# hanruihua/NeuPAN

Hardware: AMD Instinct MI355X
Metric: MPC plans/sec (node), diff robot, 1k pts, T=10, K=10; ctrl L2 vs ref (higher is better)
Workload: dtype f32; 1 GPU; BASELINE.json configs[1]: batch=256 synthetic scenes/GPU, diff robot, 1000 pts, T=10, K=10 (iter_threshold=0), M=10, fp32 DUNE (MFMA) + fp64 QP; scenes_per_gpu=256, points=1000, T=10, K=10, M=10, batches_in_flight=40, chains=8, issue_threads=8

## Files before the change

neupan_amd/csrc/dune.hip:

```cpp
#include "pan_common.h"
#include <hip/hip_ext.h>
#include <algorithm>
#include <cstdlib>
#include <cstring>
#include "dune_device.h"

static int tiles_per_slice(const DevParams& P, int n_stride) {
  int n_use_max = n_stride < P.dune_max_num ? n_stride : P.dune_max_num;
  if (n_use_max < 1) n_use_max = 1;
  return (n_use_max + 31) / 32;
}

extern "C" hipError_t npa_launch_encode(const DevParams& P, const float* wpack, int batch, int scene0, int t0,
                                        int n_stride, const float* cur_s, const float* points, const float* vel,
                                        const int* n_points, const int* flags, unsigned* gkeys, const float* trig,
                                        int n_cu, int blocks_per_cu, int key_terms, hipStream_t stream,
                                        hipEvent_t ev_start, hipEvent_t ev_stop) {
  const int nsl = P.T + 1 - t0;
  const int tps = tiles_per_slice(P, n_stride);
  if (tps * 32 > P.key_stride) return hipErrorInvalidValue;
  const long long tiles = (long long)batch * nsl * tps;
  if (tiles >= (1ll << 31)) return hipErrorInvalidValue;
  const bool split = key_terms != 0, single = key_terms == 1;
  if (!split && blocks_per_cu > 4) blocks_per_cu = 4;
  static const bool small_only = getenv("NPA_ENC_WAVES") && atoi(getenv("NPA_ENC_WAVES")) == 4;
  int waves = (split && !small_only && P.E == 4 && tiles >= (long long)n_cu * 16 * 4) ? 16 : DUNE_WAVES;
  const int slots = waves >= 8 ? n_cu : n_cu * blocks_per_cu;
  int blocks = (int)((tiles + waves - 1) / waves);
  if (blocks > slots) blocks = slots;
  if (blocks < 1) blocks = 1;
  const size_t shmem = (11 * 32 + 8 * 32 + 8) * sizeof(float) + (split ? WP_KEY_LDS_FLOATS * sizeof(float) : 0);
  static const int chunk_env = getenv("NPA_ENC_CHUNK") ? atoi(getenv("NPA_ENC_CHUNK")) : 2;
  const int chunk = chunk_env < 1 ? 1 : chunk_env;
#define LAUNCH1(EE, SP, WV)                                                                                         \
  hipExtLaunchKernelGGL((dune_kernel<EE, SP, WV>), dim3(blocks), dim3(64 * WV), shmem, stream, ev_start, ev_stop, 0, \
                        P, wpack, n_stride, cur_s, points, vel, n_points, flags, gkeys, tps * 32, scene0, batch, t0, \
                        chunk, trig)
#define LAUNCH(EE)                                                                                                  \
  do {                                                                                                              \
    if (single) LAUNCH1(EE, 1, DUNE_WAVES);                                                                         \
    else if (split) LAUNCH1(EE, 3, DUNE_WAVES);                                                                     \
    else LAUNCH1(EE, 0, DUNE_WAVES);                                                                                \
  } while (0)
#define LAUNCH16(EE)                                                                                                \
  do {                                                                                                              \
    if (single && waves == 16) LAUNCH1(EE, 1, 16);                                                                  \
    else if (split && waves == 16) LAUNCH1(EE, 3, 16);                                                              \
    else LAUNCH(EE);                                                                                                \
  } while (0)
  switch (P.E) {
    case 3: LAUNCH(3); break;
    case 4: LAUNCH16(4); break;
    case 5: LAUNCH(5); break;
    case 6: LAUNCH(6); break;
    case 7: LAUNCH(7); break;
    case 8: LAUNCH(8); break;
    default: return hipErrorInvalidValue;
  }
#undef LAUNCH16
#undef LAUNCH
#undef LAUNCH1
  return hipGetLastError();
}

extern "C" hipError_t npa_launch_select(const DevParams& P, const float* wpack, int batch, int scene0, int t0,
                                        int n_stride, const float* cur_s, const float* points, const float* vel,
                                        const int* n_points, const int* flags, const unsigned* gkeys,
                                        const float* trig, float* mu_sorted, float* lam_sorted, float* pts_sorted,
                                        float* dist_sorted, int* count, int key_terms, float e0, unsigned* stats,
                                        int debug, hipStream_t stream, hipEvent_t ev_start, hipEvent_t ev_stop) {
  const int nsl = P.T + 1 - t0;
  const int tps = tiles_per_slice(P, n_stride);
  const int dbg = debug ? 2 : 1;
  const bool geo = key_terms == 4;
  const int approx = key_terms == 0 ? 0 : dbg;
  const size_t key_area = std::max<size_t>((size_t)tps * 32 * sizeof(unsigned), SEL_CAP * (NPA_MAX_E + 5 + 2) * sizeof(float));
  const size_t shmem = (11 * 32 + 8 * 32 + 8 + NPA_GEO_BANDS) * sizeof(float) + (SEL_CAP + NPA_MAX_M + 64) * sizeof(int) +
                       (key_area + 15) / 16 * 16;
#define LAUNCH1(EE, GG)                                                                                             \
  do {                                                                                                              \
    static NpaDeviceOnce big_lds;                                                                                   \
    int dev_ = 0;                                                                                                   \
    if (shmem > 60 * 1024 && big_lds.need(&dev_)) {                                                                 \
      hipError_t e_ = hipFuncSetAttribute(reinterpret_cast<const void*>(select_kernel<EE, GG>),                     \
                                          hipFuncAttributeMaxDynamicSharedMemorySize, 160 * 1024);                  \
      if (e_ != hipSuccess) return e_;                                                                              \
      big_lds.done(dev_);                                                                                           \
    }                                                                                                               \
    hipExtLaunchKernelGGL((select_kernel<EE, GG>), dim3(nsl, batch), dim3(64), shmem, stream, ev_start, ev_stop, 0, P,    \
                          wpack, n_stride, cur_s, points, vel, n_points, flags, gkeys, tps * 32, mu_sorted, lam_sorted, \
                          pts_sorted, dist_sorted, count, scene0, t0, approx, e0, stats, trig);                      \
  } while (0)
#ifdef NPA_EXPERIMENTS
#define LAUNCH(EE)                                                                                                  \
  do {                                                                                                              \
    if (geo) LAUNCH1(EE, true);                                                                                     \
    else LAUNCH1(EE, false);                                                                                        \
  } while (0)
#else
#define LAUNCH(EE)                                                                                                  \
  do {                                                                                                              \
    if (geo) return hipErrorInvalidValue;                                                                           \
    LAUNCH1(EE, false);                                                                                             \
  } while (0)
#endif
  switch (P.E) {
    case 3: LAUNCH(3); break;
    case 4: LAUNCH(4); break;
    case 5: LAUNCH(5); break;
    case 6: LAUNCH(6); break;
    case 7: LAUNCH(7); break;
    case 8: LAUNCH(8); break;
    default: return hipErrorInvalidValue;
  }
#undef LAUNCH
#undef LAUNCH1
  return hipGetLastError();
}

extern "C" hipError_t npa_launch_select_geo(const DevParams& P, const float* wpack, int batch, int scene0, int t0,
                                            int n_stride, const float* cur_s, const float* points, const float* vel,
                                            const int* n_points, const int* flags, const float* trig, float* mu_sorted,
                                            float* lam_sorted, float* pts_sorted, float* dist_sorted, int* count,
                                            unsigned* stats, int debug, unsigned* audit, unsigned audit_thresh,
                                            unsigned audit_seed, float margin_scale, int rows_bf16, hipStream_t stream,
                                            hipEvent_t ev_start, hipEvent_t ev_stop) {
  const int nsl = P.T + 1 - t0;
  int n_use_max = n_stride < P.dune_max_num ? n_stride : P.dune_max_num;
  if (n_use_max < 1) n_use_max = 1;
  const size_t n_pad = ((size_t)n_use_max + SEL2_TRIP - 1) / SEL2_TRIP * SEL2_TRIP;
  const size_t key_area = std::max<size_t>(n_pad * sizeof(unsigned), SEL_CAP * (NPA_MAX_E + 5 + 2) * sizeof(float));
  const size_t shmem = (11 * 32 + 8 * 32 + 8 + NPA_GEO_BANDS) * sizeof(float) + (2 * SEL_CAP + NPA_MAX_M) * sizeof(int) +
                       (key_area + 15) / 16 * 16;
  const int blocks = (batch + 7) / 8 * 8 * nsl;
#define LAUNCHG(EE, BB, KK)                                                                                         \
  do {                                                                                                              \
    static NpaDeviceOnce big_lds;                                                                                   \
    int dev_ = 0;                                                                                                   \
    if (shmem > 60 * 1024 && big_lds.need(&dev_)) {                                                                 \
      hipError_t e_ = hipFuncSetAttribute(reinterpret_cast<const void*>(select_geo_kernel<EE, BB, KK>),             \
                                          hipFuncAttributeMaxDynamicSharedMemorySize, 160 * 1024);                  \
      if (e_ != hipSuccess) return e_;                                                                              \
      big_lds.done(dev_);                                                                                           \
    }                                                                                                               \
    hipExtLaunchKernelGGL((select_geo_kernel<EE, BB, KK>), dim3(blocks), dim3(64), shmem, stream, ev_start, ev_stop, 0, P, wpack,  \
                          n_stride, cur_s, points, vel, n_points, flags, mu_sorted, lam_sorted, pts_sorted, dist_sorted, \
                          count, scene0, t0, nsl, batch, debug, stats, trig, audit, audit_thresh, audit_seed, margin_scale); \
  } while (0)
#define LAUNCH(EE)                                                                                                  \
  do {                                                                                                              \
    if (rows_bf16) return hipErrorInvalidValue;                                                                     \
    LAUNCHG(EE, false, false);                                                                                      \
  } while (0)
#define LAUNCHB(EE)                                                                                                 \
  do {                                                                                                              \
    if (rows_bf16 == 1) LAUNCHG(EE, true, false);                                                                   \
    else if (rows_bf16 == 2) LAUNCHG(EE, false, true);                                                              \
    else LAUNCHG(EE, false, false);                                                                                 \
  } while (0)
  switch (P.E) {
    case 3: LAUNCH(3); break;
    case 4: LAUNCHB(4); break;
    case 5: LAUNCH(5); break;
    case 6: LAUNCH(6); break;
    case 7: LAUNCH(7); break;
    case 8: LAUNCHB(8); break;
    default: return hipErrorInvalidValue;
  }
#undef LAUNCH
#undef LAUNCHB
#undef LAUNCHG
  return hipGetLastError();
}

extern "C" hipError_t npa_launch_select_geo_group(const DevParams& P, const SelGeoGroup& G, int n, int batch, int t0, int n_stride_max,
                                                  int debug, unsigned audit_thresh, float margin_scale, int rows_bf16,
                                                  hipStream_t stream, hipEvent_t ev_start, hipEvent_t ev_stop) {
  if (n < 1 || n > NPA_GROUP_MAX) return hipErrorInvalidValue;
  const int nsl = P.T + 1 - t0;
  int n_use_max = n_stride_max < P.dune_max_num ? n_stride_max : P.dune_max_num;
  if (n_use_max < 1) n_use_max = 1;
  const size_t n_pad = ((size_t)n_use_max + SEL2_TRIP - 1) / SEL2_TRIP * SEL2_TRIP;
  const size_t key_area = std::max<size_t>(n_pad * sizeof(unsigned), SEL_CAP * (NPA_MAX_E + 5 + 2) * sizeof(float));
  const size_t shmem = (11 * 32 + 8 * 32 + 8 + NPA_GEO_BANDS) * sizeof(float) + (2 * SEL_CAP + NPA_MAX_M) * sizeof(int) +
                       (key_area + 15) / 16 * 16;
  const int blocks = (batch + 7) / 8 * 8 * nsl;
#define LAUNCHG(EE, BB, KK)                                                                                         \
  do {                                                                                                              \
    static NpaDeviceOnce big_lds;                                                                                   \
    int dev_ = 0;                                                                                                   \
    if (shmem > 60 * 1024 && big_lds.need(&dev_)) {                                                                 \
      hipError_t e_ = hipFuncSetAttribute(reinterpret_cast<const void*>(select_geo_group_kernel<EE, BB, KK>),       \
                                          hipFuncAttributeMaxDynamicSharedMemorySize, 160 * 1024);                  \
      if (e_ != hipSuccess) return e_;                                                                              \
      big_lds.done(dev_);                                                                                           \
    }                                                                                                               \
    hipExtLaunchKernelGGL((select_geo_group_kernel<EE, BB, KK>), dim3(blocks, n), dim3(64), shmem, stream, ev_start, ev_stop, 0, P, G, \
                          t0, nsl, batch, debug, audit_thresh, margin_scale);                                       \
  } while (0)
  if (rows_bf16 == 1) return hipErrorInvalidValue;
  if (P.E == 4) { if (rows_bf16 == 2) LAUNCHG(4, false, true); else LAUNCHG(4, false, false); }
  else if (P.E == 8) { if (rows_bf16 == 2) LAUNCHG(8, false, true); else LAUNCHG(8, false, false); }
  else return hipErrorInvalidValue;
#undef LAUNCHG
  return hipGetLastError();
}
extern "C" int npa_select_geo_group_supported(int E) { return E == 4 || E == 8; }

template <int E>
__global__ __launch_bounds__(256) void geo_calib_kernel(DevParams P, const float* __restrict__ wpack, float half, int nside,
                                                        float inner, float shift, unsigned* __restrict__ out) {
  extern __shared__ __attribute__((aligned(16))) float smem[];
  float* vec = smem;
  float* w6 = vec + 11 * 32;
  float* b6 = w6 + 8 * 32;
  unsigned* tab = reinterpret_cast<unsigned*>(b6 + 8);
  const int tid = threadIdx.x, lane = tid & 63, j = lane & 31, hf = lane >> 5;
  for (int i = tid; i < 11 * 32 + 8 * 32 + 8; i += blockDim.x) smem[i] = wpack[WP_VEC + i];
  for (int i = tid; i < 2 * NPA_GEO_BANDS; i += blockDim.x) tab[i] = 0u;
  __syncthreads();
  WaveWeights W;
  load_weights(wpack, lane, W);
  const float step = 2.0f * half / (float)(nside - 1);
  const int tiles_x = nside >> 3, tiles_y = nside >> 2;
  const long long tiles = (long long)tiles_x * tiles_y;
  const long long wave = (long long)blockIdx.x * (blockDim.x >> 6) + (tid >> 6), nwave = (long long)gridDim.x * (blockDim.x >> 6);
  for (long long tile = wave; tile < tiles; tile += nwave) {
    const int ix = (int)(tile % tiles_x) * 8 + (j & 7), iy = (int)(tile / tiles_x) * 4 + (j >> 3);
    const float p0x = -half + step * ((float)ix + shift), p0y = -half + step * ((float)iy + shift);
    float me[E];
    encode_tile<E>(W, vec, w6, b6, p0x, p0y, lane, me);
    float de = 0.f;
#pragma unroll
    for (int e = 0; e < E; ++e) de = fmaf(me[e], __fsub_rn(fmaf(P.G[e][0], p0x, __fmul_rn(P.G[e][1], p0y)), P.h[e]), de);
    const float g = geo_dist<E>(P, p0x, p0y);
    float f = de - g;
    if (!(f == f)) f = 3.0e38f;
    const float fx = __shfl_down(f, 1, 64), fy = __shfl_down(f, 8, 64);
    if (hf == 0 && fmaxf(fabsf(p0x), fabsf(p0y)) >= inner) {
      const int band = npa_geo_band(g);
      atomicMax(&tab[band], __float_as_uint(fabsf(f)));
      float df = 0.f;
      if ((j & 7) < 7) df = fabsf(fx - f);
      if (j < 24) df = fmaxf(df, fabsf(fy - f));
      atomicMax(&tab[NPA_GEO_BANDS + band], __float_as_uint(df));
    }
  }
  __syncthreads();
  for (int i = tid; i < 2 * NPA_GEO_BANDS; i += blockDim.x)
    if (tab[i]) atomicMax(&out[i], tab[i]);
}

extern "C" hipError_t npa_launch_geo_calib(const DevParams& P, const float* wpack, int nside, float half, float inner,
                                           float shift, unsigned* out, int n_cu, hipStream_t stream) {
  const size_t shmem = (11 * 32 + 8 * 32 + 8 + 2 * NPA_GEO_BANDS) * sizeof(float);
  const int blocks = n_cu * 4;
#define LAUNCH(EE) hipLaunchKernelGGL((geo_calib_kernel<EE>), dim3(blocks), dim3(256), shmem, stream, P, wpack, half, nside, inner, shift, out)
  switch (P.E) {
    case 3: LAUNCH(3); break;
    case 4: LAUNCH(4); break;
    case 5: LAUNCH(5); break;
    case 6: LAUNCH(6); break;
    case 7: LAUNCH(7); break;
    case 8: LAUNCH(8); break;
    default: return hipErrorInvalidValue;
  }
#undef LAUNCH
  return hipGetLastError();
}

template <int E>
__global__ __launch_bounds__(256) void k16_calib_kernel(DevParams P, const float* __restrict__ wpack, float half, int nside, float inner,
                                                        unsigned* __restrict__ out) {
  extern __shared__ __attribute__((aligned(16))) float smem[];
  float* vec = smem;
  float* w6 = vec + 11 * 32;
  float* b6 = w6 + 8 * 32;
  unsigned* tab = reinterpret_cast<unsigned*>(b6 + 8);
  const int tid = threadIdx.x, lane = tid & 63, j = lane & 31, hf = lane >> 5;
  for (int i = tid; i < 11 * 32 + 8 * 32 + 8; i += blockDim.x) smem[i] = wpack[WP_VEC + i];
  for (int i = tid; i < NPA_GEO_BANDS; i += blockDim.x) tab[i] = 0u;
  __syncthreads();
  const float w1 = wpack[WP_W1 + lane];
  const float step = 2.0f * half / (float)(nside - 1);
  const int tiles_x = nside >> 3, tiles_y = nside >> 2;
  const long long tiles = (long long)tiles_x * tiles_y;
  const long long wave = (long long)blockIdx.x * (blockDim.x >> 6) + (tid >> 6), nwave = (long long)gridDim.x * (blockDim.x >> 6);
  for (long long tile = wave; tile < tiles; tile += nwave) {
    const int ix = (int)(tile % tiles_x) * 8 + (j & 7), iy = (int)(tile / tiles_x) * 4 + (j >> 3);
    const float p0x = -half + step * (float)ix, p0y = -half + step * (float)iy;
    float me[E], mb[E];
    encode_tile_stream<E>(w1, wpack + WP_WLS, vec, w6, b6, p0x, p0y, lane, me);
    encode_tile_bf16<E>(w1, wpack + WP_WB16, vec, w6, b6, p0x, p0y, lane, mb);
    float de = 0.f, db = 0.f;
#pragma unroll
    for (int e = 0; e < E; ++e) {
      const float tmp = __fsub_rn(fmaf(P.G[e][0], p0x, __fmul_rn(P.G[e][1], p0y)), P.h[e]);
      de = fmaf(me[e], tmp, de);
      db = fmaf(mb[e], tmp, db);
    }
    float f = fabsf(db - de);
    if (!(f == f)) f = 3.0e38f;
    if (hf == 0 && fmaxf(fabsf(p0x), fabsf(p0y)) >= inner) atomicMax(&tab[npa_geo_band(de)], __float_as_uint(f));
  }
  __syncthreads();
  for (int i = tid; i < NPA_GEO_BANDS; i += blockDim.x)
    if (tab[i]) atomicMax(&out[i], tab[i]);
}
extern "C" hipError_t npa_launch_k16_calib(const DevParams& P, const float* wpack, int nside, float half, float inner, unsigned* out,
                                           int n_cu, hipStream_t stream) {
  const size_t shmem = (11 * 32 + 8 * 32 + 8 + NPA_GEO_BANDS) * sizeof(float);
  const int blocks = n_cu * 4;
  if (P.E == 4) hipLaunchKernelGGL((k16_calib_kernel<4>), dim3(blocks), dim3(256), shmem, stream, P, wpack, half, nside, inner, out);
  else if (P.E == 8) hipLaunchKernelGGL((k16_calib_kernel<8>), dim3(blocks), dim3(256), shmem, stream, P, wpack, half, nside, inner, out);
  else return hipErrorInvalidValue;
  return hipGetLastError();
}

template <int E>
__global__ __launch_bounds__(256) void geo_table_nodes_kernel(DevParams P, const float* __restrict__ wpack, float* __restrict__ nodes) {
  extern __shared__ __attribute__((aligned(16))) float smem[];
  float* vec = smem;
  float* w6 = vec + 11 * 32;
  float* b6 = w6 + 8 * 32;
  const int tid = threadIdx.x, lane = tid & 63, j = lane & 31, hf = lane >> 5;
  for (int i = tid; i < 11 * 32 + 8 * 32 + 8; i += blockDim.x) smem[i] = wpack[WP_VEC + i];
  __syncthreads();
  const float w1 = wpack[WP_W1 + lane];
  constexpr int nside = NPA_TAB_N + 1, per = nside * nside, total = NPA_TAB_LEVELS * per;
  const int tiles = (total + 31) / 32;
  const int wave = blockIdx.x * (blockDim.x >> 6) + (tid >> 6), nwave = gridDim.x * (blockDim.x >> 6);
  for (int tile = wave; tile < tiles; tile += nwave) {
    const int n = tile * 32 + j, nc = n < total ? n : total - 1;
    const int lvl = nc / per, r = nc - lvl * per, iy = r / nside, ix = r - iy * nside;
    const float half = wpack[WP_TABH + 2] * (lvl == 0 ? 1.0f : (lvl == 1 ? 4.0f : (lvl == 2 ? 16.0f : 64.0f)));
    const float step = 2.0f * half / (float)NPA_TAB_N;
    const float p0x = wpack[WP_TABH] + fmaf(step, (float)ix, -half), p0y = wpack[WP_TABH + 1] + fmaf(step, (float)iy, -half);
    float me[E];
    encode_tile_stream<E>(w1, wpack + WP_WLS, vec, w6, b6, p0x, p0y, lane, me);
    float de = 0.f;
#pragma unroll
    for (int e = 0; e < E; ++e) de = fmaf(me[e], __fsub_rn(fmaf(P.G[e][0], p0x, __fmul_rn(P.G[e][1], p0y)), P.h[e]), de);
    if (hf == 0 && n < total) nodes[n] = de - geo_key<E>(P, p0x, p0y);
  }
}
__global__ void geo_table_pack_kernel(const float* __restrict__ nodes, float* __restrict__ wpack) {
  const int c = blockIdx.x * blockDim.x + threadIdx.x;
  constexpr int N = NPA_TAB_N, nside = N + 1;
  if (c >= NPA_TAB_LEVELS * N * N) return;
  const int lvl = c / (N * N), r = c - lvl * N * N, iy = r / N, ix = r - iy * N;
  const float* nl = nodes + (size_t)lvl * nside * nside;
  typedef _Float16 h2_t __attribute__((ext_vector_type(2)));
  union { unsigned u; h2_t h; } lo, hi;
  lo.h[0] = (_Float16)nl[iy * nside + ix]; lo.h[1] = (_Float16)nl[iy * nside + ix + 1];
  hi.h[0] = (_Float16)nl[(iy + 1) * nside + ix]; hi.h[1] = (_Float16)nl[(iy + 1) * nside + ix + 1];
  reinterpret_cast<uint2*>(wpack + WP_TAB)[c] = make_uint2(lo.u, hi.u);
}
extern "C" hipError_t npa_launch_geo_table(const DevParams& P, float* wpack, float* nodes, int n_cu, hipStream_t stream) {
  const size_t shmem = (11 * 32 + 8 * 32 + 8) * sizeof(float);
  const int blocks = n_cu * 4;
#define LAUNCH(EE) hipLaunchKernelGGL((geo_table_nodes_kernel<EE>), dim3(blocks), dim3(256), shmem, stream, P, wpack, nodes)
  switch (P.E) {
    case 4: LAUNCH(4); break;
    case 8: LAUNCH(8); break;
    default: return hipErrorInvalidValue;
  }
#undef LAUNCH
  hipError_t e = hipGetLastError();
  if (e != hipSuccess) return e;
  const int cells = NPA_TAB_LEVELS * NPA_TAB_N * NPA_TAB_N;
  hipLaunchKernelGGL(geo_table_pack_kernel, dim3((cells + 255) / 256), dim3(256), 0, stream, nodes, wpack);
  return hipGetLastError();
}
template <int E>
__global__ __launch_bounds__(256) void ktab_calib_kernel(DevParams P, const float* __restrict__ wpack, float half, int nside, float inner,
                                                         float cx, float cy, unsigned* __restrict__ out) {
  extern __shared__ __attribute__((aligned(16))) float smem[];
  float* vec = smem;
  float* w6 = vec + 11 * 32;
  float* b6 = w6 + 8 * 32;
  unsigned* tab = reinterpret_cast<unsigned*>(b6 + 8);
  const int tid = threadIdx.x, lane = tid & 63, j = lane & 31, hf = lane >> 5;
  for (int i = tid; i < 11 * 32 + 8 * 32 + 8; i += blockDim.x) smem[i] = wpack[WP_VEC + i];
  for (int i = tid; i < NPA_GEO_BANDS; i += blockDim.x) tab[i] = 0u;
  __syncthreads();
  const float w1 = wpack[WP_W1 + lane];
  const float step = 2.0f * half / (float)(nside - 1);
  const int tiles_x = nside >> 3, tiles_y = nside >> 2;
  const long long tiles = (long long)tiles_x * tiles_y;
  const long long wave = (long long)blockIdx.x * (blockDim.x >> 6) + (tid >> 6), nwave = (long long)gridDim.x * (blockDim.x >> 6);
  for (long long tile = wave; tile < tiles; tile += nwave) {
    const int ix = (int)(tile % tiles_x) * 8 + (j & 7), iy = (int)(tile / tiles_x) * 4 + (j >> 3);
    const float qx = -half + step * (float)ix, qy = -half + step * (float)iy;
    const float p0x = cx + qx, p0y = cy + qy;
    float me[E];
    encode_tile_stream<E>(w1, wpack + WP_WLS, vec, w6, b6, p0x, p0y, lane, me);
    float de = 0.f;
#pragma unroll
    for (int e = 0; e < E; ++e) de = fmaf(me[e], __fsub_rn(fmaf(P.G[e][0], p0x, __fmul_rn(P.G[e][1], p0y)), P.h[e]), de);
    const float kc = geo_key<E>(P, p0x, p0y) + geo_tab_corr(wpack, p0x, p0y);
    float f = fabsf(kc - de);
    if (!(f == f)) f = 3.0e38f;
    if (hf == 0 && fmaxf(fabsf(qx), fabsf(qy)) >= inner) atomicMax(&tab[npa_geo_band(kc)], __float_as_uint(f));
  }
  __syncthreads();
  for (int i = tid; i < NPA_GEO_BANDS; i += blockDim.x)
    if (tab[i]) atomicMax(&out[i], tab[i]);
}
extern "C" hipError_t npa_launch_ktab_calib(const DevParams& P, const float* wpack, int nside, float half, float inner, float cx, float cy,
                                            unsigned* out, int n_cu, hipStream_t stream) {
  const size_t shmem = (11 * 32 + 8 * 32 + 8 + NPA_GEO_BANDS) * sizeof(float);
  const int blocks = n_cu * 4;
#define LAUNCH(EE) hipLaunchKernelGGL((ktab_calib_kernel<EE>), dim3(blocks), dim3(256), shmem, stream, P, wpack, half, nside, inner, cx, cy, out)
  switch (P.E) {
    case 4: LAUNCH(4); break;
    case 8: LAUNCH(8); break;
    default: return hipErrorInvalidValue;
  }
#undef LAUNCH
  return hipGetLastError();
}

template <int E, int TERMS>
__global__ __launch_bounds__(256) void key_calib_kernel(DevParams P, const float* __restrict__ wpack, float lo, float step,
                                                        int nside, unsigned* __restrict__ out) {
  extern __shared__ __attribute__((aligned(16))) float smem[];
  float* vec = smem;
  float* w6 = vec + 11 * 32;
  float* b6 = w6 + 8 * 32;
  float* wb = b6 + 8;
  const int tid = threadIdx.x, lane = tid & 63, j = lane & 31, hf = lane >> 5;
  for (int i = tid; i < 11 * 32 + 8 * 32 + 8; i += blockDim.x) smem[i] = wpack[WP_VEC + i];
  for (int i = tid; i < WP_KEY_LDS_FLOATS; i += blockDim.x) wb[i] = wpack[WP_BF + i];
  __syncthreads();
  const f16x8* wbf = reinterpret_cast<const f16x8*>(wb);
  WaveWeights W;
  load_weights(wpack, lane, W);
  const float kw1 = wpack[WP_KW1 + lane];
  const int tile = blockIdx.x * (blockDim.x >> 6) + (tid >> 6);
  const int n = tile * 32 + j, total = nside * nside;
  const int nc = n < total ? n : total - 1;
  const float p0x = lo + step * (float)(nc % nside), p0y = lo + step * (float)(nc / nside);
  float mk[E], me[E];
  encode_tile_keys<E, TERMS>(kw1, wbf, vec, w6, b6, p0x, p0y, lane, mk);
  encode_tile<E>(W, vec, w6, b6, p0x, p0y, lane, me);
  float dk = 0.f, de = 0.f;
#pragma unroll
  for (int e = 0; e < E; ++e) {
    const float tmp = __fsub_rn(fmaf(P.G[e][0], p0x, __fmul_rn(P.G[e][1], p0y)), P.h[e]);
    dk = e < P.E ? fmaf(mk[e], tmp, dk) : dk;
    de = e < P.E ? fmaf(me[e], tmp, de) : de;
  }
  float rel = fabsf(dk - de) / (1.0f + fabsf(de));
  if (!(rel == rel)) rel = 1e30f;
  if (hf == 0 && n < total) atomicMax(out, __float_as_uint(rel));
}

extern "C" hipError_t npa_launch_key_calib(const DevParams& P, const float* wpack, int key_terms, int nside, float half,
                                           unsigned* out, hipStream_t stream) {
  const int tiles = (nside * nside + 31) / 32, blocks = (tiles + 3) / 4;
  const float lo = -half, step = 2.0f * half / (float)(nside - 1);
  const size_t shmem = (11 * 32 + 8 * 32 + 8 + WP_KEY_LDS_FLOATS) * sizeof(float);
#define LAUNCH(EE)                                                                                                   \
  do {                                                                                                               \
    if (key_terms == 1) hipLaunchKernelGGL((key_calib_kernel<EE, 1>), dim3(blocks), dim3(256), shmem, stream, P, wpack, lo, step, nside, out); \
    else hipLaunchKernelGGL((key_calib_kernel<EE, 3>), dim3(blocks), dim3(256), shmem, stream, P, wpack, lo, step, nside, out); \
  } while (0)
  if (P.E < 3 || P.E > NPA_MAX_E) return hipErrorInvalidValue;
  LAUNCH(NPA_MAX_E);
#undef LAUNCH
  return hipGetLastError();
}

__global__ void trig_kernel(const float* __restrict__ cur_s, int nscene, int T, float* __restrict__ trig) {
  const int i = blockIdx.x * blockDim.x + threadIdx.x;
  if (i >= nscene * (T + 1)) return;
  const int b = i / (T + 1), t = i - b * (T + 1);
  float c, s;
  npa_trig(cur_s[(size_t)b * 3 * (T + 1) + 2 * (T + 1) + t], c, s);
  trig[2 * (size_t)i] = c;
  trig[2 * (size_t)i + 1] = s;
}
extern "C" hipError_t npa_launch_trig(const float* cur_s, int batch, int T, float* trig, hipStream_t stream) {
  const int n = batch * (T + 1);
  hipLaunchKernelGGL(trig_kernel, dim3((n + 255) / 256), dim3(256), 0, stream, cur_s, batch, T, trig);
  return hipGetLastError();
}
```

neupan_amd/csrc/dune_device.h:

```cpp
#pragma once

typedef float f32x16 __attribute__((ext_vector_type(16)));

#define DUNE_THREADS 256
#define DUNE_WAVES 4

#define WSYNC()                                              \
  do {                                                       \
    __builtin_amdgcn_fence(__ATOMIC_SEQ_CST, "wavefront");   \
    __builtin_amdgcn_wave_barrier();                         \
  } while (0)

__device__ __forceinline__ float pair_sum(float x) {
  auto r = __builtin_amdgcn_permlane32_swap(__float_as_uint(x), __float_as_uint(x), false, false);
  return __uint_as_float(r[0]) + __uint_as_float(r[1]);
}

__device__ __forceinline__ float tanh_scaled(float y) {
  float e = __builtin_amdgcn_exp2f(y);
  return fmaf(-2.0f, __builtin_amdgcn_rcpf(e + 1.0f), 1.0f);
}

__device__ __forceinline__ void load_vec16(const float* v, int hf, float out[16]) {
#pragma unroll
  for (int q = 0; q < 4; ++q) {
    float4 t = *reinterpret_cast<const float4*>(v + 8 * q + 4 * hf);
    out[4 * q + 0] = t.x; out[4 * q + 1] = t.y; out[4 * q + 2] = t.z; out[4 * q + 3] = t.w;
  }
}

template <bool PERM>
__device__ __forceinline__ void load_vec16x(const float* v, int hf, float out[16]) {
  if constexpr (!PERM) {
    load_vec16(v, hf, out);
  } else {
#pragma unroll
    for (int h2 = 0; h2 < 2; ++h2)
#pragma unroll
      for (int qq = 0; qq < 2; ++qq) {
        const float4 t = *reinterpret_cast<const float4*>(v + 16 * h2 + 8 * hf + 4 * qq);
        out[2 * (4 * qq + 0) + h2] = t.x; out[2 * (4 * qq + 1) + h2] = t.y; out[2 * (4 * qq + 2) + h2] = t.z; out[2 * (4 * qq + 3) + h2] = t.w;
      }
  }
}
template <bool PERM = false>
__device__ __forceinline__ f32x16 bias_init(const float* v, int hf) {
  float b[16];
  load_vec16x<PERM>(v, hf, b);
  f32x16 acc;
#pragma unroll
  for (int r = 0; r < 16; ++r) acc[r] = b[r];
  return acc;
}

typedef float f32x4 __attribute__((ext_vector_type(4)));
__device__ __forceinline__ float quad_sum(float x) {
  auto r = __builtin_amdgcn_permlane16_swap(__float_as_uint(x), __float_as_uint(x), false, false);
  return pair_sum(__uint_as_float(r[0]) + __uint_as_float(r[1]));
}

template <bool PERM = false>
__device__ __forceinline__ void ln_tanh(f32x16 acc, const float* g, const float* be, int hf, float a[16]) {
  float se = acc[0], so = acc[1];
#pragma unroll
  for (int r = 2; r < 16; r += 2) { se += acc[r]; so += acc[r + 1]; }
  float mean = (pair_sum(se) + pair_sum(so)) * (1.0f / 32.0f);
  float qe = 0.f, qo = 0.f;
#pragma unroll
  for (int r = 0; r < 16; r += 2) {
    a[r] = acc[r] - mean; qe = fmaf(a[r], a[r], qe);
    a[r + 1] = acc[r + 1] - mean; qo = fmaf(a[r + 1], a[r + 1], qo);
  }
  float var = (pair_sum(qe) + pair_sum(qo)) * (1.0f / 32.0f);
  float ve = var + 1e-5f;
  float rstd = __builtin_amdgcn_rsqf(ve);
  rstd = rstd * fmaf(-0.5f * ve * rstd, rstd, 1.5f);
  if constexpr (PERM) {
#pragma unroll
    for (int h2 = 0; h2 < 2; ++h2)
#pragma unroll
      for (int qq = 0; qq < 2; ++qq) {
        const float4 gv = *reinterpret_cast<const float4*>(g + 16 * h2 + 8 * hf + 4 * qq);
        const float4 bv = *reinterpret_cast<const float4*>(be + 16 * h2 + 8 * hf + 4 * qq);
        const int r0 = 2 * (4 * qq) + h2;
        a[r0 + 0] = tanh_scaled(fmaf(a[r0 + 0] * rstd, gv.x, bv.x));
        a[r0 + 2] = tanh_scaled(fmaf(a[r0 + 2] * rstd, gv.y, bv.y));
        a[r0 + 4] = tanh_scaled(fmaf(a[r0 + 4] * rstd, gv.z, bv.z));
        a[r0 + 6] = tanh_scaled(fmaf(a[r0 + 6] * rstd, gv.w, bv.w));
      }
    return;
  }
#pragma unroll
  for (int qd = 0; qd < 4; ++qd) {
    float4 gv = *reinterpret_cast<const float4*>(g + 8 * qd + 4 * hf);
    float4 bv = *reinterpret_cast<const float4*>(be + 8 * qd + 4 * hf);
    a[4 * qd + 0] = tanh_scaled(fmaf(a[4 * qd + 0] * rstd, gv.x, bv.x));
    a[4 * qd + 1] = tanh_scaled(fmaf(a[4 * qd + 1] * rstd, gv.y, bv.y));
    a[4 * qd + 2] = tanh_scaled(fmaf(a[4 * qd + 2] * rstd, gv.z, bv.z));
    a[4 * qd + 3] = tanh_scaled(fmaf(a[4 * qd + 3] * rstd, gv.w, bv.w));
  }
}

__device__ __forceinline__ f32x16 layer32(const float (&w)[16], const float (&a)[16], f32x16 acc) {
#pragma unroll
  for (int r = 0; r < 16; ++r) acc = __builtin_amdgcn_mfma_f32_32x32x2f32(w[r], a[r], acc, 0, 0, 0);
  return acc;
}

typedef _Float16 f16x8 __attribute__((ext_vector_type(8)));
typedef _Float16 f16x2 __attribute__((ext_vector_type(2)));
typedef float f32x2_t __attribute__((ext_vector_type(2)));


template <bool RELU>
__device__ __forceinline__ void split2(const float (&a)[16], f16x8 (&x1)[2], f16x8 (&x2)[2]) {
#pragma unroll
  for (int p = 0; p < 8; ++p) {
    f32x2_t v = {a[2 * p], a[2 * p + 1]};
    if constexpr (RELU) {
      v.x = __int_as_float(max(__float_as_int(v.x), 0));
      v.y = __int_as_float(max(__float_as_int(v.y), 0));
    }
    const f16x2 b1 = __builtin_convertvector(v, f16x2);
    const f32x2_t r1 = v - __builtin_convertvector(b1, f32x2_t);
    const f16x2 b2 = __builtin_convertvector(r1, f16x2);
    const int s = p >> 2, q = (2 * p) & 7;
    x1[s][q] = b1.x; x1[s][q + 1] = b1.y;
    x2[s][q] = b2.x; x2[s][q + 1] = b2.y;
  }
}

template <bool RELU, int TERMS>
__device__ __forceinline__ f32x16 layer32_f16x2(const f16x8* wl, int lane, const float (&a)[16], f32x16 acc) {
  if constexpr (TERMS == 1) {
    f16x8 x[2];
#pragma unroll
    for (int p = 0; p < 8; ++p) {
      f16x2 b1 = __builtin_convertvector(f32x2_t{a[2 * p], a[2 * p + 1]}, f16x2);
      if constexpr (RELU) b1 = __builtin_elementwise_max(b1, f16x2{(_Float16)0.f, (_Float16)0.f});
      const int s = p >> 2, q = (2 * p) & 7;
      x[s][q] = b1.x; x[s][q + 1] = b1.y;
    }
#pragma unroll
    for (int s = 0; s < 2; ++s) acc = __builtin_amdgcn_mfma_f32_32x32x16_f16(wl[(0 * 2 + s) * 64 + lane], x[s], acc, 0, 0, 0);
    return acc;
  }
  f16x8 x1[2], x2[2];
  split2<RELU>(a, x1, x2);
#pragma unroll
  for (int s = 0; s < 2; ++s) {
    const f16x8 w1 = wl[(0 * 2 + s) * 64 + lane], w2 = wl[(1 * 2 + s) * 64 + lane];
    acc = __builtin_amdgcn_mfma_f32_32x32x16_f16(w2, x1[s], acc, 0, 0, 0);
    acc = __builtin_amdgcn_mfma_f32_32x32x16_f16(w1, x2[s], acc, 0, 0, 0);
    acc = __builtin_amdgcn_mfma_f32_32x32x16_f16(w1, x1[s], acc, 0, 0, 0);
  }
  return acc;
}

typedef float f32x2 __attribute__((ext_vector_type(2)));

__device__ __forceinline__ void ln_tanh_centred(f32x16 acc, const float* g, const float* be, int hf, float eps,
                                                float out_scale, float a[16]) {
  f32x2 q2 = {0.f, 0.f};
#pragma unroll
  for (int p = 0; p < 8; ++p) {
    const f32x2 v = {acc[2 * p], acc[2 * p + 1]};
    q2 = __builtin_elementwise_fma(v, v, q2);
  }
  const float ve = fmaf(pair_sum(q2.x + q2.y), 1.0f / 32.0f, eps);
  float rstd = __builtin_amdgcn_rsqf(ve);
  rstd = rstd * fmaf(-0.5f * ve * rstd, rstd, 1.5f);
  const f32x2 rs = {rstd, rstd}, one = {1.f, 1.f}, osc = {out_scale, out_scale}, mtwo = {-2.f * out_scale, -2.f * out_scale};
#pragma unroll
  for (int qd = 0; qd < 4; ++qd) {
    const float4 gv = *reinterpret_cast<const float4*>(g + 8 * qd + 4 * hf);
    const float4 bv = *reinterpret_cast<const float4*>(be + 8 * qd + 4 * hf);
#pragma unroll
    for (int hh = 0; hh < 2; ++hh) {
      const f32x2 x = {acc[4 * qd + 2 * hh], acc[4 * qd + 2 * hh + 1]};
      const f32x2 gg = hh ? f32x2{gv.z, gv.w} : f32x2{gv.x, gv.y};
      const f32x2 bb = hh ? f32x2{bv.z, bv.w} : f32x2{bv.x, bv.y};
      const f32x2 y = __builtin_elementwise_fma(x * rs, gg, bb);
      f32x2 e = {__builtin_amdgcn_exp2f(y.x), __builtin_amdgcn_exp2f(y.y)};
      e = e + one;
      const f32x2 r = {__builtin_amdgcn_rcpf(e.x), __builtin_amdgcn_rcpf(e.y)};
      const f32x2 th = __builtin_elementwise_fma(r, mtwo, osc);
      a[4 * qd + 2 * hh] = th.x; a[4 * qd + 2 * hh + 1] = th.y;
    }
  }
}

template <int E, int TERMS>
__device__ __forceinline__ void encode_tile_keys(float kw1, const f16x8* wbf, const float* vec, const float* w6,
                                                 const float* b6, float p0x, float p0y, int lane, float mu[E]) {
  const int hf = lane >> 5;
  const float* kvec = reinterpret_cast<const float*>(wbf) + WP_BF_FLOATS;
  const float* ksc = kvec + 5 * 32;
  constexpr int LSTR = 2 * 2 * 64;
  float a[16];
  {
    f32x16 acc = bias_init(kvec + 0 * 32, hf);
    acc = __builtin_amdgcn_mfma_f32_32x32x2f32(kw1, hf ? p0y : p0x, acc, 0, 0, 0);
    ln_tanh_centred(acc, vec + V_G1 * 32, vec + V_BE1 * 32, hf, ksc[0], ksc[3], a);
  }
  {
    f32x16 acc = layer32_f16x2<false, TERMS>(wbf + 0 * LSTR, lane, a, bias_init(kvec + 1 * 32, hf));
#pragma unroll
    for (int r = 0; r < 16; ++r) a[r] = acc[r];
  }
  {
    f32x16 acc = layer32_f16x2<true, TERMS>(wbf + 1 * LSTR, lane, a, bias_init(kvec + 2 * 32, hf));
    ln_tanh_centred(acc, vec + V_G2 * 32, vec + V_BE2 * 32, hf, ksc[1], ksc[4], a);
  }
  {
    f32x16 acc = layer32_f16x2<false, TERMS>(wbf + 2 * LSTR, lane, a, bias_init(kvec + 3 * 32, hf));
#pragma unroll
    for (int r = 0; r < 16; ++r) a[r] = acc[r];
  }
  {
    f32x16 acc = layer32_f16x2<true, TERMS>(wbf + 3 * LSTR, lane, a, bias_init(kvec + 4 * 32, hf));
    ln_tanh_centred(acc, vec + V_G3 * 32, vec + V_BE3 * 32, hf, ksc[2], ksc[5], a);
  }
#pragma unroll
  for (int e = 0; e < E; ++e) {
    float wv[16];
    load_vec16(w6 + e * 32, hf, wv);
    f32x2 s2 = {0.f, 0.f};
#pragma unroll
    for (int p = 0; p < 8; ++p)
      s2 = __builtin_elementwise_fma(f32x2{wv[2 * p], wv[2 * p + 1]}, f32x2{a[2 * p], a[2 * p + 1]}, s2);
    mu[e] = fmaxf(pair_sum(s2.x + s2.y) + b6[e], 0.f);
  }
}

struct WaveWeights {
  float w1;
  float wl[4][16];
};

template <int E>
__device__ __forceinline__ void encode_tile(const WaveWeights& W, const float* vec, const float* w6, const float* b6,
                                            float p0x, float p0y, int lane, float mu[E]) {
  const int hf = lane >> 5;
  auto layer = [&](int L, const float (&a_)[16], f32x16 acc) -> f32x16 { return layer32(W.wl[L], a_, acc); };
  float a[16];
  {
    f32x16 acc = bias_init(vec + V_B1 * 32, hf);
    acc = __builtin_amdgcn_mfma_f32_32x32x2f32(W.w1, hf ? p0y : p0x, acc, 0, 0, 0);
    ln_tanh(acc, vec + V_G1 * 32, vec + V_BE1 * 32, hf, a);
  }
  {
    f32x16 acc = layer(0, a, bias_init(vec + V_B2 * 32, hf));
#pragma unroll
    for (int r = 0; r < 16; ++r) a[r] = fmaxf(acc[r], 0.f);
  }
  {
    f32x16 acc = layer(1, a, bias_init(vec + V_B3 * 32, hf));
    ln_tanh(acc, vec + V_G2 * 32, vec + V_BE2 * 32, hf, a);
  }
  {
    f32x16 acc = layer(2, a, bias_init(vec + V_B4 * 32, hf));
#pragma unroll
    for (int r = 0; r < 16; ++r) a[r] = fmaxf(acc[r], 0.f);
  }
  {
    f32x16 acc = layer(3, a, bias_init(vec + V_B5 * 32, hf));
    ln_tanh(acc, vec + V_G3 * 32, vec + V_BE3 * 32, hf, a);
  }
#pragma unroll
  for (int e = 0; e < E; ++e) {
    float wv[16];
    load_vec16(w6 + e * 32, hf, wv);
    float se = 0.f, so = 0.f;
#pragma unroll
    for (int r = 0; r < 16; r += 2) { se = fmaf(wv[r], a[r], se); so = fmaf(wv[r + 1], a[r + 1], so); }
    mu[e] = fmaxf((pair_sum(se) + pair_sum(so)) + b6[e], 0.f);
  }
}

__device__ __forceinline__ void load_layer(const float* __restrict__ wls, int L, int lane, float (&w)[16]) {
  asm volatile("" : "+v"(lane));
  const float4* p = reinterpret_cast<const float4*>(wls + ((size_t)L * 64 + lane) * 16);
#pragma unroll
  for (int q = 0; q < 4; ++q) {
    const float4 v = p[q];
    w[4 * q] = v.x; w[4 * q + 1] = v.y; w[4 * q + 2] = v.z; w[4 * q + 3] = v.w;
  }
}
template <int E, bool PERM = false>
__device__ __forceinline__ void encode_tile_stream(float w1, const float* __restrict__ wls, const float* vec, const float* w6,
                                                   const float* b6, float p0x, float p0y, int lane, float mu[E]) {
  int hf = lane >> 5;
  if constexpr (PERM) asm volatile("" : "+v"(hf));
  float a[16], wa[16], wb[16];
  load_layer(wls, 0, lane, wa);
  __builtin_amdgcn_sched_barrier(0);
  {
    f32x16 acc = bias_init<PERM>(vec + V_B1 * 32, hf);
    acc = __builtin_amdgcn_mfma_f32_32x32x2f32(w1, hf ? p0y : p0x, acc, 0, 0, 0);
    ln_tanh<PERM>(acc, vec + V_G1 * 32, vec + V_BE1 * 32, hf, a);
  }
  __builtin_amdgcn_sched_barrier(0);
  load_layer(wls, 1, lane, wb);
  __builtin_amdgcn_sched_barrier(0);
  {
    f32x16 acc = layer32(wa, a, bias_init<PERM>(vec + V_B2 * 32, hf));
#pragma unroll
    for (int r = 0; r < 16; ++r) a[r] = fmaxf(acc[r], 0.f);
  }
  __builtin_amdgcn_sched_barrier(0);
  load_layer(wls, 2, lane, wa);
  __builtin_amdgcn_sched_barrier(0);
  {
    f32x16 acc = layer32(wb, a, bias_init<PERM>(vec + V_B3 * 32, hf));
    ln_tanh<PERM>(acc, vec + V_G2 * 32, vec + V_BE2 * 32, hf, a);
  }
  __builtin_amdgcn_sched_barrier(0);
  load_layer(wls, 3, lane, wb);
  __builtin_amdgcn_sched_barrier(0);
  {
    f32x16 acc = layer32(wa, a, bias_init<PERM>(vec + V_B4 * 32, hf));
#pragma unroll
    for (int r = 0; r < 16; ++r) a[r] = fmaxf(acc[r], 0.f);
  }
  __builtin_amdgcn_sched_barrier(0);
  {
    f32x16 acc = layer32(wb, a, bias_init<PERM>(vec + V_B5 * 32, hf));
    ln_tanh<PERM>(acc, vec + V_G3 * 32, vec + V_BE3 * 32, hf, a);
  }
  __builtin_amdgcn_sched_barrier(0);
#pragma unroll
  for (int e = 0; e < E; ++e) {
    float wv[16];
    load_vec16x<PERM>(w6 + e * 32, hf, wv);
    float se = 0.f, so = 0.f;
#pragma unroll
    for (int r = 0; r < 16; r += 2) { se = fmaf(wv[r], a[r], se); so = fmaf(wv[r + 1], a[r + 1], so); }
    mu[e] = fmaxf((pair_sum(se) + pair_sum(so)) + b6[e], 0.f);
  }
}

__device__ __forceinline__ f32x4 ld4(const float* p) {
  const float4 t = *reinterpret_cast<const float4*>(p);
  return f32x4{t.x, t.y, t.z, t.w};
}
__device__ __forceinline__ void ln_tanh16(f32x4 c0, f32x4 c1, const float* g, const float* be, int kq, float a[8]) {
  float s = c0[0];
  s += c0[1]; s += c0[2]; s += c0[3]; s += c1[0]; s += c1[1]; s += c1[2]; s += c1[3];
  const float mean = quad_sum(s) * (1.0f / 32.0f);
  float q = 0.f;
#pragma unroll
  for (int r = 0; r < 4; ++r) { a[r] = c0[r] - mean; q = fmaf(a[r], a[r], q); }
#pragma unroll
  for (int r = 0; r < 4; ++r) { a[4 + r] = c1[r] - mean; q = fmaf(a[4 + r], a[4 + r], q); }
  const float var = quad_sum(q) * (1.0f / 32.0f);
  const float ve = var + 1e-5f;
  float rstd = __builtin_amdgcn_rsqf(ve);
  rstd = rstd * fmaf(-0.5f * ve * rstd, rstd, 1.5f);
#pragma unroll
  for (int qd = 0; qd < 2; ++qd) {
    const float4 gv = *reinterpret_cast<const float4*>(g + 8 * kq + 4 * qd);
    const float4 bv = *reinterpret_cast<const float4*>(be + 8 * kq + 4 * qd);
    a[4 * qd + 0] = tanh_scaled(fmaf(a[4 * qd + 0] * rstd, gv.x, bv.x));
    a[4 * qd + 1] = tanh_scaled(fmaf(a[4 * qd + 1] * rstd, gv.y, bv.y));
    a[4 * qd + 2] = tanh_scaled(fmaf(a[4 * qd + 2] * rstd, gv.z, bv.z));
    a[4 * qd + 3] = tanh_scaled(fmaf(a[4 * qd + 3] * rstd, gv.w, bv.w));
  }
}
__device__ __forceinline__ void layer16(const float (&w)[16], const float (&a)[8], f32x4& c0, f32x4& c1) {
#pragma unroll
  for (int s = 0; s < 8; ++s) {
    c0 = __builtin_amdgcn_mfma_f32_16x16x4f32(w[2 * s], a[s], c0, 0, 0, 0);
    c1 = __builtin_amdgcn_mfma_f32_16x16x4f32(w[2 * s + 1], a[s], c1, 0, 0, 0);
  }
}
template <int E>
__device__ __forceinline__ void encode_tile16_stream(float w1a, float w1b, const float* __restrict__ wls16, const float* vec,
                                                     const float* w6, const float* b6, float p0x, float p0y, int lane, float mu[E]) {
  int kq = lane >> 4;
  asm volatile("" : "+v"(kq));
  const float* vq = vec + 8 * kq;
  float a[8], wa[16], wb[16];
  load_layer(wls16, 0, lane, wa);
  __builtin_amdgcn_sched_barrier(0);
  {
    f32x4 c0 = ld4(vq + V_B1 * 32), c1 = ld4(vq + V_B1 * 32 + 4);
    const float bx = kq == 0 ? p0x : (kq == 1 ? p0y : 0.f);
    c0 = __builtin_amdgcn_mfma_f32_16x16x4f32(w1a, bx, c0, 0, 0, 0);
    c1 = __builtin_amdgcn_mfma_f32_16x16x4f32(w1b, bx, c1, 0, 0, 0);
    ln_tanh16(c0, c1, vec + V_G1 * 32, vec + V_BE1 * 32, kq, a);
  }
  __builtin_amdgcn_sched_barrier(0);
  load_layer(wls16, 1, lane, wb);
  __builtin_amdgcn_sched_barrier(0);
  {
    f32x4 c0 = ld4(vq + V_B2 * 32), c1 = ld4(vq + V_B2 * 32 + 4);
    layer16(wa, a, c0, c1);
#pragma unroll
    for (int r = 0; r < 4; ++r) { a[r] = fmaxf(c0[r], 0.f); a[4 + r] = fmaxf(c1[r], 0.f); }
  }
  __builtin_amdgcn_sched_barrier(0);
  load_layer(wls16, 2, lane, wa);
  __builtin_amdgcn_sched_barrier(0);
  {
    f32x4 c0 = ld4(vq + V_B3 * 32), c1 = ld4(vq + V_B3 * 32 + 4);
    layer16(wb, a, c0, c1);
    ln_tanh16(c0, c1, vec + V_G2 * 32, vec + V_BE2 * 32, kq, a);
  }
  __builtin_amdgcn_sched_barrier(0);
  load_layer(wls16, 3, lane, wb);
  __builtin_amdgcn_sched_barrier(0);
  {
    f32x4 c0 = ld4(vq + V_B4 * 32), c1 = ld4(vq + V_B4 * 32 + 4);
    layer16(wa, a, c0, c1);
#pragma unroll
    for (int r = 0; r < 4; ++r) { a[r] = fmaxf(c0[r], 0.f); a[4 + r] = fmaxf(c1[r], 0.f); }
  }
  __builtin_amdgcn_sched_barrier(0);
  {
    f32x4 c0 = ld4(vq + V_B5 * 32), c1 = ld4(vq + V_B5 * 32 + 4);
    layer16(wb, a, c0, c1);
    ln_tanh16(c0, c1, vec + V_G3 * 32, vec + V_BE3 * 32, kq, a);
  }
  __builtin_amdgcn_sched_barrier(0);
#pragma unroll
  for (int e = 0; e < E; ++e) {
    const f32x4 w0 = ld4(w6 + e * 32 + 8 * kq), w1 = ld4(w6 + e * 32 + 8 * kq + 4);
    float s = 0.f;
#pragma unroll
    for (int r = 0; r < 4; ++r) s = fmaf(w0[r], a[r], s);
#pragma unroll
    for (int r = 0; r < 4; ++r) s = fmaf(w1[r], a[4 + r], s);
    mu[e] = fmaxf(quad_sum(s) + b6[e], 0.f);
  }
}

typedef __bf16 bf16x8 __attribute__((ext_vector_type(8)));
typedef __bf16 bf16x2 __attribute__((ext_vector_type(2)));
__device__ __forceinline__ f32x16 layer32_bf16(const bf16x8* __restrict__ wb, int L, int lane, const float (&a)[16], f32x16 acc) {
  bf16x8 x[2];
#pragma unroll
  for (int p = 0; p < 8; ++p) {
    const bf16x2 b = __builtin_convertvector(f32x2_t{a[2 * p], a[2 * p + 1]}, bf16x2);
    const int s = p >> 2, q = (2 * p) & 7;
    x[s][q] = b.x; x[s][q + 1] = b.y;
  }
#pragma unroll
  for (int s = 0; s < 2; ++s) acc = __builtin_amdgcn_mfma_f32_32x32x16_bf16(wb[(L * 2 + s) * 64 + lane], x[s], acc, 0, 0, 0);
  return acc;
}
template <int E>
__device__ __forceinline__ void encode_tile_bf16(float w1, const float* __restrict__ wb16, const float* vec, const float* w6,
                                                 const float* b6, float p0x, float p0y, int lane, float mu[E]) {
  const int hf = lane >> 5;
  const bf16x8* wb = reinterpret_cast<const bf16x8*>(wb16);
  float a[16];
  {
    f32x16 acc = bias_init(vec + V_B1 * 32, hf);
    acc = __builtin_amdgcn_mfma_f32_32x32x2f32(w1, hf ? p0y : p0x, acc, 0, 0, 0);
    ln_tanh(acc, vec + V_G1 * 32, vec + V_BE1 * 32, hf, a);
  }
  {
    f32x16 acc = layer32_bf16(wb, 0, lane, a, bias_init(vec + V_B2 * 32, hf));
#pragma unroll
    for (int r = 0; r < 16; ++r) a[r] = fmaxf(acc[r], 0.f);
  }
  {
    f32x16 acc = layer32_bf16(wb, 1, lane, a, bias_init(vec + V_B3 * 32, hf));
    ln_tanh(acc, vec + V_G2 * 32, vec + V_BE2 * 32, hf, a);
  }
  {
    f32x16 acc = layer32_bf16(wb, 2, lane, a, bias_init(vec + V_B4 * 32, hf));
#pragma unroll
    for (int r = 0; r < 16; ++r) a[r] = fmaxf(acc[r], 0.f);
  }
  {
    f32x16 acc = layer32_bf16(wb, 3, lane, a, bias_init(vec + V_B5 * 32, hf));
    ln_tanh(acc, vec + V_G3 * 32, vec + V_BE3 * 32, hf, a);
  }
#pragma unroll
  for (int e = 0; e < E; ++e) {
    float wv[16];
    load_vec16(w6 + e * 32, hf, wv);
    float se = 0.f, so = 0.f;
#pragma unroll
    for (int r = 0; r < 16; r += 2) { se = fmaf(wv[r], a[r], se); so = fmaf(wv[r + 1], a[r + 1], so); }
    mu[e] = fmaxf((pair_sum(se) + pair_sum(so)) + b6[e], 0.f);
  }
}

__device__ __forceinline__ unsigned ordered_key(float d) {
  if (d != d) return 0xFFFFFFFEu;
  unsigned b = __float_as_uint(d);
  return (b & 0x80000000u) ? ~b : (b | 0x80000000u);
}

template <int CTRL>
__device__ __forceinline__ unsigned long long dpp_u64(unsigned long long v) {
  unsigned lo = (unsigned)__builtin_amdgcn_update_dpp(0, (int)(unsigned)v, CTRL, 0xF, 0xF, false);
  unsigned hi = (unsigned)__builtin_amdgcn_update_dpp(0, (int)(unsigned)(v >> 32), CTRL, 0xF, 0xF, false);
  return ((unsigned long long)hi << 32) | lo;
}
__device__ __forceinline__ unsigned long long umin64(unsigned long long a, unsigned long long b) { return a < b ? a : b; }
__device__ __forceinline__ unsigned long long readlane_u64(unsigned long long v, int l) {
  unsigned lo = __builtin_amdgcn_readlane((unsigned)v, l), hi = __builtin_amdgcn_readlane((unsigned)(v >> 32), l);
  return ((unsigned long long)hi << 32) | lo;
}
__device__ __forceinline__ unsigned long long wave_min_u64(unsigned long long v) {
  v = umin64(v, dpp_u64<0xB1>(v));
  v = umin64(v, dpp_u64<0x4E>(v));
  v = umin64(v, dpp_u64<0x141>(v));
  v = umin64(v, dpp_u64<0x140>(v));
  return umin64(umin64(readlane_u64(v, 0), readlane_u64(v, 16)), umin64(readlane_u64(v, 32), readlane_u64(v, 48)));
}

struct SliceFrame {
  float c, s, tx, ty;
  float tstep;
  float rg[2][NPA_MAX_E];
};

__device__ __forceinline__ int src_index(int n, int n_raw, int n_use) {
  if (n_use >= n_raw) return n;
  if (n == n_use - 1) return n_raw - 1;
  double step = (double)(n_raw - 1) / (double)(n_use - 1);
  return (int)((double)n * step);
}

template <int E>
__device__ __forceinline__ void load_frame(const DevParams& P, const float* __restrict__ cur_s,
                                           const float* __restrict__ trig, int b, int t, SliceFrame& F) {
  const int T = P.T;
  const float* s = cur_s + (size_t)b * 3 * (T + 1);
  F.tx = s[t];
  F.ty = s[(T + 1) + t];
  F.c = trig[((size_t)b * (T + 1) + t) * 2];
  F.s = trig[((size_t)b * (T + 1) + t) * 2 + 1];
  F.tstep = (float)t;
#pragma unroll
  for (int e = 0; e < E; ++e) {
    F.rg[0][e] = fmaf(-F.c, P.G[e][0], __fmul_rn(F.s, P.G[e][1]));
    F.rg[1][e] = fmaf(-F.s, P.G[e][0], -__fmul_rn(F.c, P.G[e][1]));
  }
  auto uni = [](float v) { return __uint_as_float(__builtin_amdgcn_readfirstlane(__float_as_uint(v))); };
  F.c = uni(F.c); F.s = uni(F.s); F.tx = uni(F.tx); F.ty = uni(F.ty); F.tstep = uni(F.tstep);
#pragma unroll
  for (int e = 0; e < E; ++e) { F.rg[0][e] = uni(F.rg[0][e]); F.rg[1][e] = uni(F.rg[1][e]); }
}

template <int E, int SPLIT>
__device__ __forceinline__ void point_features(const DevParams& P, const SliceFrame& F, const WaveWeights& W,
                                               const f16x8* wbf, const float* vec, const float* w6, const float* b6,
                                               const float* px_row, const float* py_row, const float* vx_row,
                                               const float* vy_row, int src, int lane, float mu[E], float& gx,
                                               float& gy, float& lx, float& ly, float& dist) {
  gx = px_row[src];
  gy = py_row[src];
  if (vx_row) {
    gx = __fadd_rn(gx, __fmul_rn(F.tstep, __fmul_rn(vx_row[src], P.dt32)));
    gy = __fadd_rn(gy, __fmul_rn(F.tstep, __fmul_rn(vy_row[src], P.dt32)));
  }
  float dx = __fsub_rn(gx, F.tx), dy = __fsub_rn(gy, F.ty);
  float p0x = fmaf(F.c, dx, __fmul_rn(F.s, dy));
  float p0y = fmaf(F.c, dy, -__fmul_rn(F.s, dx));
  if constexpr (SPLIT != 0) encode_tile_keys<E, SPLIT>(W.w1, wbf, vec, w6, b6, p0x, p0y, lane, mu);
  else encode_tile<E>(W, vec, w6, b6, p0x, p0y, lane, mu);
  lx = 0.f; ly = 0.f; dist = 0.f;
#pragma unroll
  for (int e = 0; e < E; ++e) {
    lx = fmaf(F.rg[0][e], mu[e], lx);
    ly = fmaf(F.rg[1][e], mu[e], ly);
    float tmp = __fsub_rn(fmaf(P.G[e][0], p0x, __fmul_rn(P.G[e][1], p0y)), P.h[e]);
    dist = fmaf(mu[e], tmp, dist);
  }
}

template <int E, bool BF16 = false, bool PERM = false>
__device__ __forceinline__ void point_features_stream(const DevParams& P, const SliceFrame& F, float w1, const float* __restrict__ wls,
                                                      const float* vec, const float* w6, const float* b6, const float* px_row,
                                                      const float* py_row, const float* vx_row, const float* vy_row, int src,
                                                      int lane, float mu[E], float& gx, float& gy, float& lx, float& ly,
                                                      float& dist, float& p0x, float& p0y) {
  gx = px_row[src];
  gy = py_row[src];
  if (vx_row) {
    gx = __fadd_rn(gx, __fmul_rn(F.tstep, __fmul_rn(vx_row[src], P.dt32)));
    gy = __fadd_rn(gy, __fmul_rn(F.tstep, __fmul_rn(vy_row[src], P.dt32)));
  }
  float dx = __fsub_rn(gx, F.tx), dy = __fsub_rn(gy, F.ty);
  p0x = fmaf(F.c, dx, __fmul_rn(F.s, dy));
  p0y = fmaf(F.c, dy, -__fmul_rn(F.s, dx));
  if constexpr (BF16) encode_tile_bf16<E>(w1, wls, vec, w6, b6, p0x, p0y, lane, mu);
  else encode_tile_stream<E, PERM>(w1, wls, vec, w6, b6, p0x, p0y, lane, mu);
  lx = 0.f; ly = 0.f; dist = 0.f;
#pragma unroll
  for (int e = 0; e < E; ++e) {
    lx = fmaf(F.rg[0][e], mu[e], lx);
    ly = fmaf(F.rg[1][e], mu[e], ly);
    float tmp = __fsub_rn(fmaf(P.G[e][0], p0x, __fmul_rn(P.G[e][1], p0y)), P.h[e]);
    dist = fmaf(mu[e], tmp, dist);
  }
}

template <int E>
__device__ __forceinline__ void point_features_stream16(const DevParams& P, const SliceFrame& F, float w1a, float w1b,
                                                        const float* __restrict__ wls16, const float* vec, const float* w6,
                                                        const float* b6, const float* px_row, const float* py_row,
                                                        const float* vx_row, const float* vy_row, int src, int lane, float mu[E],
                                                        float& gx, float& gy, float& lx, float& ly, float& dist, float& p0x,
                                                        float& p0y) {
  gx = px_row[src];
  gy = py_row[src];
  if (vx_row) {
    gx = __fadd_rn(gx, __fmul_rn(F.tstep, __fmul_rn(vx_row[src], P.dt32)));
    gy = __fadd_rn(gy, __fmul_rn(F.tstep, __fmul_rn(vy_row[src], P.dt32)));
  }
  float dx = __fsub_rn(gx, F.tx), dy = __fsub_rn(gy, F.ty);
  p0x = fmaf(F.c, dx, __fmul_rn(F.s, dy));
  p0y = fmaf(F.c, dy, -__fmul_rn(F.s, dx));
  encode_tile16_stream<E>(w1a, w1b, wls16, vec, w6, b6, p0x, p0y, lane, mu);
  lx = 0.f; ly = 0.f; dist = 0.f;
#pragma unroll
  for (int e = 0; e < E; ++e) {
    lx = fmaf(F.rg[0][e], mu[e], lx);
    ly = fmaf(F.rg[1][e], mu[e], ly);
    float tmp = __fsub_rn(fmaf(P.G[e][0], p0x, __fmul_rn(P.G[e][1], p0y)), P.h[e]);
    dist = fmaf(mu[e], tmp, dist);
  }
}

__device__ __forceinline__ void load_weights(const float* __restrict__ wpack, int lane, WaveWeights& W) {
  W.w1 = wpack[WP_W1 + lane];
#pragma unroll
  for (int l = 0; l < 4; ++l)
#pragma unroll
    for (int r = 0; r < 16; ++r) W.wl[l][r] = wpack[WP_WL + (l * 16 + r) * 64 + lane];
}

template <int E, int SPLIT, int WAVES>
__global__ __attribute__((amdgpu_flat_work_group_size(64 * WAVES, 64 * WAVES), amdgpu_waves_per_eu(WAVES >= 8 ? 7 : ((SPLIT == 0 && E >= 6) ? 3 : 4))))
void dune_kernel(
    DevParams P, const float* __restrict__ wpack, int n_stride, const float* __restrict__ cur_s,
    const float* __restrict__ points, const float* __restrict__ vel, const int* __restrict__ n_points,
    const int* __restrict__ flags, unsigned* __restrict__ gkeys, int key_stride, int scene0, int nscene, int t0,
    int chunk, const float* __restrict__ trig) {
  extern __shared__ __attribute__((aligned(16))) float smem[];
  __shared__ int wg_ticket_s;
  int* wg_ticket = &wg_ticket_s;
  if (threadIdx.x == 0) wg_ticket_s = 0;
  float* vec = smem;
  float* w6 = vec + 11 * 32;
  float* b6 = w6 + 8 * 32;
  const int tid = threadIdx.x, lane = tid & 63;
  const int wave = __builtin_amdgcn_readfirstlane(tid >> 6);
  const int j = lane & 31, hf = lane >> 5;
  const int T = P.T;

  for (int i = tid; i < 11 * 32 + 8 * 32 + 8; i += 64 * WAVES) smem[i] = wpack[WP_VEC + i];
  WaveWeights W;
  const f16x8* wbf = nullptr;
  if constexpr (SPLIT != 0) {
    float* wb = b6 + 8;
    for (int i = tid; i < WP_KEY_LDS_FLOATS; i += 64 * WAVES) wb[i] = wpack[WP_BF + i];
    wbf = reinterpret_cast<const f16x8*>(wb);
    W.w1 = wpack[WP_KW1 + lane];
  } else {
    load_weights(wpack, lane, W);
  }
  __syncthreads();

  const int nsl = T + 1 - t0;
  const int tps = key_stride >> 5;
  const int total = nscene * nsl * tps;
  const int wg_lo = (int)((long long)total * blockIdx.x / gridDim.x);
  const int wg_hi = (int)((long long)total * (blockIdx.x + 1) / gridDim.x);
  int g = 0, hi = 0, sl = 0, tile = 0;
  int cur_sl = -1, n_raw = 0, n_use = 0, t = 0;
  bool skip = false;
  SliceFrame F;
  const float *px_row = nullptr, *py_row = nullptr, *vx_row = nullptr, *vy_row = nullptr;
  unsigned* key_row = nullptr;
#pragma unroll 1
  for (;; ++g, ++tile) {
    if (g >= hi) {
      int c = 0;
      if (lane == 0) c = atomicAdd(wg_ticket, chunk);
      g = wg_lo + __builtin_amdgcn_readfirstlane(c);
      if (g >= wg_hi) break;
      hi = g + chunk < wg_hi ? g + chunk : wg_hi;
      sl = (int)((unsigned)g / (unsigned)tps);
      tile = g - sl * tps;
    } else if (tile == tps) {
      tile = 0;
      ++sl;
    }
    if (sl != cur_sl) {
      cur_sl = sl;
      const int bl = (int)((unsigned)sl / (unsigned)nsl), b = bl + scene0;
      t = sl - bl * nsl + t0;
      n_raw = n_points ? n_points[b] : n_stride;
      n_raw = n_raw < 0 ? 0 : (n_raw > n_stride ? n_stride : n_raw);
      n_use = n_raw < P.dune_max_num ? n_raw : P.dune_max_num;
      skip = (flags && flags[b * 4 + 0]) || n_use <= 0;
      if (!skip) {
        load_frame<E>(P, cur_s, trig, b, t, F);
        px_row = points + (size_t)b * 2 * n_stride;
        py_row = px_row + n_stride;
        vx_row = vel ? vel + (size_t)b * 2 * n_stride : nullptr;
        vy_row = vel ? vx_row + n_stride : nullptr;
        key_row = gkeys + ((size_t)b * (T + 1) + t) * key_stride;
      }
    }
    if (skip || tile * 32 >= n_use) continue;
    {
      const int n = tile * 32 + j;
      const int nc = n < n_use ? n : n_use - 1;
      float mu[E], gx, gy, lx, ly, dist;
      point_features<E, SPLIT>(P, F, W, wbf, vec, w6, b6, px_row, py_row, vx_row, vy_row, src_index(nc, n_raw, n_use),
                               lane, mu, gx, gy, lx, ly, dist);
      if (hf == 0 && n < n_use) key_row[n] = ordered_key(dist);
    }
  }
}

template <int E>
__device__ __forceinline__ float geo_dist(const DevParams& P, float x, float y) {
  if (P.geo_rect) {
    const float dx = fmaxf(fabsf(x - P.rcx) - P.rhx, 0.f), dy = fmaxf(fabsf(y - P.rcy) - P.rhy, 0.f);
    return __builtin_sqrtf(fmaf(dx, dx, dy * dy));
  }
  float best = 3.0e38f;
  bool inside = true;
#pragma unroll
  for (int e = 0; e < E; ++e) {
    const float rx = x - P.pvx[e], ry = y - P.pvy[e];
    inside = inside && (fmaf(P.pdy[e], rx, -(P.pdx[e] * ry)) <= 0.f);
    float t = fmaf(rx, P.pdx[e], ry * P.pdy[e]) * P.pil[e];
    t = fminf(fmaxf(t, 0.f), 1.f);
    const float qx = fmaf(-t, P.pdx[e], rx), qy = fmaf(-t, P.pdy[e], ry);
    best = fminf(best, fmaf(qx, qx, qy * qy));
  }
  return inside ? 0.f : __builtin_sqrtf(best);
}

#define SEL_CAP 64
template <int E, bool GEO>
__global__ __attribute__((amdgpu_flat_work_group_size(64, 64), amdgpu_waves_per_eu(E <= 6 ? 4 : 3, E <= 6 ? 4 : 3))) void select_kernel(
    DevParams P, const float* __restrict__ wpack, int n_stride, const float* __restrict__ cur_s,
    const float* __restrict__ points, const float* __restrict__ vel, const int* __restrict__ n_points,
    const int* __restrict__ flags, const unsigned* __restrict__ gkeys, int key_stride,
    float* __restrict__ mu_sorted, float* __restrict__ lam_sorted, float* __restrict__ pts_sorted,
    float* __restrict__ dist_sorted, int* __restrict__ count, int scene0, int t0, int approx_keys, float e0,
    unsigned* __restrict__ stats, const float* __restrict__ trig) {
  extern __shared__ __attribute__((aligned(16))) float smem[];
  float* vec = smem;
  float* w6 = vec + 11 * 32;
  float* b6 = w6 + 8 * 32;
  float* etab = b6 + 8;
  int* sel = reinterpret_cast<int*>(etab + NPA_GEO_BANDS);
  unsigned* skey = reinterpret_cast<unsigned*>(sel + SEL_CAP);
  int* lst = reinterpret_cast<int*>(skey + NPA_MAX_M);
  constexpr int ROW_W = E + 5;
  unsigned* dkey = reinterpret_cast<unsigned*>(lst + 64);
  float* rows = reinterpret_cast<float*>(dkey);
  unsigned* rkey = reinterpret_cast<unsigned*>(rows + SEL_CAP * (NPA_MAX_E + 5));
  const int t = blockIdx.x + t0, b = blockIdx.y + scene0, lane = threadIdx.x;
  const int j = lane & 31, hf = lane >> 5;
  const int T = P.T, M = P.M;
  if (flags && flags[b * 4 + 0]) return;
  int n_raw = n_points ? n_points[b] : n_stride;
  n_raw = n_raw < 0 ? 0 : (n_raw > n_stride ? n_stride : n_raw);
  const int n_use = n_raw < P.dune_max_num ? n_raw : P.dune_max_num;
  const size_t orow = (size_t)b * (T + 1) + t;
  if (n_use <= 0) {
    if (lane == 0) count[orow] = 0;
    return;
  }
  for (int i = lane; i < 11 * 32 + 8 * 32 + 8; i += 64) smem[i] = wpack[WP_VEC16 + i];
  if constexpr (GEO)
    for (int i = lane; i < NPA_GEO_BANDS; i += 64) etab[i] = wpack[WP_GEO + i];
  SliceFrame F;
  load_frame<E>(P, cur_s, trig, b, t, F);
  const float* px_row = points + (size_t)b * 2 * n_stride;
  const float* py_row = px_row + n_stride;
  const float* vx_row = vel ? vel + (size_t)b * 2 * n_stride : nullptr;
  const float* vy_row = vel ? vx_row + n_stride : nullptr;
  if constexpr (GEO) {
    constexpr int KU = 4;
    auto key_of = [&](float gx, float gy, float vx, float vy) -> unsigned {
      if (vx_row) {
        gx = __fadd_rn(gx, __fmul_rn(F.tstep, __fmul_rn(vx, P.dt32)));
        gy = __fadd_rn(gy, __fmul_rn(F.tstep, __fmul_rn(vy, P.dt32)));
      }
      const float dx = __fsub_rn(gx, F.tx), dy = __fsub_rn(gy, F.ty);
      const float p0x = fmaf(F.c, dx, __fmul_rn(F.s, dy)), p0y = fmaf(F.c, dy, -__fmul_rn(F.s, dx));
      const bool calibrated = fmaxf(fabsf(p0x), fabsf(p0y)) <= P.geo_rcal;
      return calibrated ? __float_as_uint(geo_dist<E>(P, p0x, p0y)) : NPA_GEO_KEY_FAR;
    };
    for (int n0 = lane; n0 < n_use; n0 += 64 * KU) {
      float gx[KU], gy[KU], vx[KU], vy[KU];
#pragma unroll
      for (int u = 0; u < KU; ++u) {
        const int n = n0 + 64 * u;
        const int src = src_index(n < n_use ? n : n_use - 1, n_raw, n_use);
        gx[u] = px_row[src]; gy[u] = py_row[src];
        vx[u] = vx_row ? vx_row[src] : 0.f; vy[u] = vy_row ? vy_row[src] : 0.f;
      }
#pragma unroll
      for (int u = 0; u < KU; ++u) {
        const int n = n0 + 64 * u;
        if (n < n_use) dkey[n] = key_of(gx[u], gy[u], vx[u], vy[u]);
      }
    }
  } else {
    const unsigned* gk = gkeys + orow * key_stride;
    for (int n = lane; n < n_use; n += 64) dkey[n] = gk[n];
  }
  const float w1a = wpack[WP_W116 + lane], w1b = wpack[WP_W116 + 64 + lane];
  const float* wls16 = wpack + WP_WL16;
  WSYNC();

  const int msel = n_use < M ? n_use : M;
  unsigned last_key = 0;
  auto extract = [&]() {
    for (int m = 0; m < msel; ++m) {
      unsigned long long best = ~0ull;
      for (int n = lane; n < n_use; n += 64) best = umin64(best, ((unsigned long long)dkey[n] << 32) | (unsigned)n);
      best = wave_min_u64(best);
      const int idx = (int)(best & 0xFFFFFFFFu);
      last_key = (unsigned)(best >> 32);
      if (lane == 0) { sel[m] = idx; skey[m] = last_key; dkey[idx] = 0xFFFFFFFFu; }
      WSYNC();
    }
  };
  auto extract_short = [&]() -> bool {
    unsigned lmin = 0xFFFFFFFFu;
    for (int n = lane; n < n_use; n += 64) lmin = min(lmin, dkey[n]);
    unsigned bound = 0;
    for (int bit = 31; bit >= 0; --bit) {
      const unsigned trial = bound | ((1u << bit) - 1u);
      if (__popcll(__ballot(lmin <= trial)) < msel) bound |= 1u << bit;
    }
    int L = 0;
    for (int n0 = 0; n0 < n_use; n0 += 64) {
      const int n = n0 + lane;
      const bool hit = n < n_use && dkey[n] <= bound;
      const unsigned long long bal = __ballot(hit);
      const int pos = L + __builtin_amdgcn_mbcnt_hi((unsigned)(bal >> 32), __builtin_amdgcn_mbcnt_lo((unsigned)bal, 0));
      if (hit && pos < 64) lst[pos] = n;
      L += __popcll(bal);
    }
    if (L > 64 || L < msel) return false;
    WSYNC();
    const int idx = lane < L ? lst[lane] : 0;
    const unsigned long long v = lane < L ? (((unsigned long long)dkey[idx] << 32) | (unsigned)idx) : ~0ull;
    int rk = 0;
    for (int i = 0; i < L; ++i) rk += readlane_u64(v, i) < v ? 1 : 0;
    if (lane < L && rk < msel) { sel[rk] = idx; skey[rk] = (unsigned)(v >> 32); dkey[idx] = 0xFFFFFFFFu; }
    const unsigned long long lastb = __ballot(lane < L && rk == msel - 1);
    last_key = (unsigned)(readlane_u64(v, (int)__builtin_ctzll(lastb)) >> 32);
    WSYNC();
    return true;
  };
  if (!extract_short()) extract();
  int ncand = msel, fellback = 0;
  bool widen = false;
  unsigned thr = 0;
  float U = 0.f;
  if constexpr (GEO) {
    widen = n_use > msel;
    float hi = -1.f;
    if (lane < msel) {
      const unsigned k = skey[lane];
      const float g = __uint_as_float(k);
      hi = (k == NPA_GEO_KEY_FAR) ? __builtin_inff() : g + etab[npa_geo_band(g)];
    }
    for (int i = 0; i < msel; ++i) U = fmaxf(U, __uint_as_float(__builtin_amdgcn_readlane(__float_as_uint(hi), i)));
  } else {
    widen = approx_keys && msel == M && n_use > M && last_key < 0xFFFFFFFEu;
    if (widen) {
      const float dM = __uint_as_float((last_key & 0x80000000u) ? (last_key & 0x7FFFFFFFu) : ~last_key);
      thr = ordered_key(dM + 2.0f * e0 * (1.0f + fabsf(dM)));
    }
  }
  bool overflow = false, all = false;
  int total = 0, extra = 0;
  if (widen) {
    for (int n0 = 0; n0 < n_use; n0 += 64) {
      const int n = n0 + lane;
      bool hit = false;
      if (n < n_use) {
        const unsigned k = dkey[n];
        if constexpr (GEO) {
          const float g = __uint_as_float(k);
          hit = k != 0xFFFFFFFFu && (k == NPA_GEO_KEY_FAR || g - etab[npa_geo_band(g)] <= U);
        } else {
          hit = k <= thr;
        }
      }
      const unsigned long long bal = __ballot(hit);
      const int pos = extra + __builtin_amdgcn_mbcnt_hi((unsigned)(bal >> 32), __builtin_amdgcn_mbcnt_lo((unsigned)bal, 0));
      if (hit) dkey[pos] = (unsigned)n;
      extra += __popcll(bal);
    }
    WSYNC();
    if (msel + extra <= SEL_CAP) {
      if (lane < extra) sel[msel + lane] = (int)dkey[lane];
      ncand = msel + extra;
      WSYNC();
    } else {
      overflow = true;
      fellback = 1;
      all = 2 * extra + msel > n_use;
      total = all ? n_use : msel + extra;
    }
  }
  unsigned* ckey = dkey + extra;
  auto cand_index = [&](int q) { return all ? q : (q < msel ? sel[q] : (int)dkey[q - msel]); };
#pragma unroll 1
  for (int phase = overflow ? 0 : 1;; phase = 1) {
    const int cnt = phase == 0 ? total : ncand;
#pragma unroll 1
    for (int q0 = 0; q0 < cnt; q0 += 16) {
      const int q = q0 + (lane & 15), qc = q < cnt ? q : cnt - 1;
      const int idx = phase == 0 ? cand_index(qc) : sel[qc];
      float mu[E], gx, gy, lx, ly, dist, p0x, p0y;
      point_features_stream16<E>(P, F, w1a, w1b, wls16, vec, w6, b6, px_row, py_row, vx_row, vy_row,
                                 src_index(idx, n_raw, n_use), lane, mu, gx, gy, lx, ly, dist, p0x, p0y);
      if (lane < 16 && q < cnt) {
        const unsigned k = ordered_key(dist);
        if (phase == 0) {
          if (all) dkey[idx] = k;
          else ckey[q] = k;
        } else {
          float* r = rows + q * ROW_W;
#pragma unroll
          for (int e = 0; e < E; ++e) r[e] = mu[e];
          r[E] = lx; r[E + 1] = ly; r[E + 2] = gx; r[E + 3] = gy; r[E + 4] = dist;
          rkey[2 * q] = (unsigned)idx; rkey[2 * q + 1] = k;
        }
      }
    }
    WSYNC();
    if (phase == 1) break;
    if (stats && lane == 0) atomicAdd(stats, (unsigned)((total + 31) / 32));
    if (all) {
      extract();
    } else {
      int mywin = 0;
      for (int m2 = 0; m2 < msel; ++m2) {
        unsigned long long best = ~0ull;
        int bq = -1;
        for (int q = lane; q < total; q += 64) {
          const unsigned long long v = ((unsigned long long)ckey[q] << 32) | (unsigned)cand_index(q);
          if (v < best) { best = v; bq = q; }
        }
        const unsigned long long win = wave_min_u64(best);
        if (best == win && bq >= 0) ckey[bq] = 0xFFFFFFFFu;
        if (lane == m2) mywin = (int)(win & 0xFFFFFFFFu);
        WSYNC();
      }
      if (lane < msel) sel[lane] = mywin;
      WSYNC();
    }
    ncand = msel;
  }
  const bool mine = lane < ncand;
  const unsigned long long kx = mine ? (((unsigned long long)rkey[2 * lane + 1] << 32) | rkey[2 * lane]) : ~0ull;
  int rank = 0;
  for (int i = 0; i < ncand; ++i) rank += readlane_u64(kx, i) < kx ? 1 : 0;
  if (mine && rank < msel) {
    const float* r = rows + lane * ROW_W;
    auto put = [&](int q) {
      const size_t o = orow * M + q;
#pragma unroll
      for (int e = 0; e < E; ++e) mu_sorted[o * E + e] = r[e];
      lam_sorted[o * 2 + 0] = r[E]; lam_sorted[o * 2 + 1] = r[E + 1];
      pts_sorted[o * 2 + 0] = r[E + 2]; pts_sorted[o * 2 + 1] = r[E + 3];
      dist_sorted[o] = r[E + 4];
    };
    put(rank);
    if (rank == 0)
      for (int q = msel; q < M; ++q) put(q);
  }
  if (lane == 0) count[orow] = approx_keys == 2 ? (msel | (ncand << 8) | (fellback << 16)) : msel;
}

__device__ __forceinline__ float dpp_f32_b1(float v) { return __int_as_float(__builtin_amdgcn_update_dpp(0, __float_as_int(v), 0xB1, 0xF, 0xF, false)); }
__device__ __forceinline__ float wave_max_f32(float v) {
  v = fmaxf(v, dpp_f32_b1(v));
  v = fmaxf(v, __int_as_float(__builtin_amdgcn_update_dpp(0, __float_as_int(v), 0x4E, 0xF, 0xF, false)));
  v = fmaxf(v, __int_as_float(__builtin_amdgcn_update_dpp(0, __float_as_int(v), 0x141, 0xF, 0xF, false)));
  v = fmaxf(v, __int_as_float(__builtin_amdgcn_update_dpp(0, __float_as_int(v), 0x140, 0xF, 0xF, false)));
  auto rl = [&](int l) { return __uint_as_float(__builtin_amdgcn_readlane(__float_as_uint(v), l)); };
  return fmaxf(fmaxf(rl(0), rl(16)), fmaxf(rl(32), rl(48)));
}
template <int E, bool RECT>
__device__ __forceinline__ float geo_key_t(const DevParams& P, float x, float y) {
  if constexpr (RECT) {
    const float dx = fmaxf(fabsf(x - P.rcx) - P.rhx, 0.f), dy = fmaxf(fabsf(y - P.rcy) - P.rhy, 0.f);
    return __builtin_amdgcn_sqrtf(fmaf(dx, dx, dy * dy));
  } else {
    float best = 3.0e38f;
    bool inside = true;
#pragma unroll
    for (int e = 0; e < E; ++e) {
      const float rx = x - P.pvx[e], ry = y - P.pvy[e];
      inside = inside && (fmaf(P.pdy[e], rx, -(P.pdx[e] * ry)) <= 0.f);
      float t = fmaf(rx, P.pdx[e], ry * P.pdy[e]) * P.pil[e];
      t = fminf(fmaxf(t, 0.f), 1.f);
      const float qx = fmaf(-t, P.pdx[e], rx), qy = fmaf(-t, P.pdy[e], ry);
      best = fminf(best, fmaf(qx, qx, qy * qy));
    }
    return inside ? 0.f : __builtin_amdgcn_sqrtf(best);
  }
}
template <int E>
__device__ __forceinline__ float geo_key(const DevParams& P, float x, float y) {
  return P.geo_rect ? geo_key_t<E, true>(P, x, y) : geo_key_t<E, false>(P, x, y);
}

__device__ __forceinline__ float geo_tab_corr(const float* __restrict__ wpack, float x, float y) {
  const float cx = wpack[WP_TABH], cy = wpack[WP_TABH + 1], h0 = wpack[WP_TABH + 2], inv0 = wpack[WP_TABH + 3];
  const float rx = x - cx, ry = y - cy;
  const float a = fmaxf(fabsf(rx), fabsf(ry));
  const int lvl = a < h0 ? 0 : (a < 4.0f * h0 ? 1 : (a < 16.0f * h0 ? 2 : 3));
  const float sc = lvl == 0 ? 1.0f : (lvl == 1 ? 4.0f : (lvl == 2 ? 16.0f : 64.0f));
  const float half = h0 * sc, inv = inv0 * (1.0f / sc);
  const float fx = fminf(fmaxf((rx + half) * inv, 0.f), (float)NPA_TAB_N - 0.001f);
  const float fy = fminf(fmaxf((ry + half) * inv, 0.f), (float)NPA_TAB_N - 0.001f);
  const int ix = (int)fx, iy = (int)fy;
  const float tx = fx - (float)ix, ty = fy - (float)iy;
  const uint2 c = reinterpret_cast<const uint2*>(wpack + WP_TAB)[((size_t)lvl * NPA_TAB_N + iy) * NPA_TAB_N + ix];
  typedef _Float16 h2_t __attribute__((ext_vector_type(2)));
  union { unsigned u; h2_t h; } lo, hi;
  lo.u = c.x; hi.u = c.y;
  const float f00 = (float)lo.h[0], f10 = (float)lo.h[1], f01 = (float)hi.h[0], f11 = (float)hi.h[1];
  const float r0 = fmaf(tx, f10 - f00, f00), r1 = fmaf(tx, f11 - f01, f01);
  return fmaf(ty, r1 - r0, r0);
}

#define SEL2_TRIP 256
template <int E, bool RECT, bool VEL, bool DEC>
__device__ __forceinline__ unsigned key_pass(const DevParams& P, const SliceFrame& F, const float* px_row, const float* py_row,
                                             const float* vx_row, const float* vy_row, unsigned* dkey, int n_raw, int n_use,
                                             int n_pad, int lane) {
  const __amdgpu_buffer_rsrc_t rx = __builtin_amdgcn_make_buffer_rsrc(const_cast<float*>(px_row), 0, n_raw * 4, 0x00020000);
  const __amdgpu_buffer_rsrc_t ry = __builtin_amdgcn_make_buffer_rsrc(const_cast<float*>(py_row), 0, n_raw * 4, 0x00020000);
  const __amdgpu_buffer_rsrc_t rvx = __builtin_amdgcn_make_buffer_rsrc(const_cast<float*>(VEL ? vx_row : px_row), 0, n_raw * 4, 0x00020000);
  const __amdgpu_buffer_rsrc_t rvy = __builtin_amdgcn_make_buffer_rsrc(const_cast<float*>(VEL ? vy_row : py_row), 0, n_raw * 4, 0x00020000);
  const float tdt = F.tstep;
  unsigned lmin = 0xFFFFFFFFu;
  for (int n0 = 0; n0 < n_pad; n0 += SEL2_TRIP) {
    float gx[4], gy[4], vx[4], vy[4];
#pragma unroll
    for (int u = 0; u < 4; ++u) {
      const int n = n0 + lane + 64 * u;
      unsigned off = (unsigned)n * 4u;
      if constexpr (DEC) off = (unsigned)src_index(n < n_use ? n : n_use - 1, n_raw, n_use) * 4u;
      gx[u] = __uint_as_float(__builtin_amdgcn_raw_buffer_load_b32(rx, off, 0, 0));
      gy[u] = __uint_as_float(__builtin_amdgcn_raw_buffer_load_b32(ry, off, 0, 0));
      if constexpr (VEL) {
        vx[u] = __uint_as_float(__builtin_amdgcn_raw_buffer_load_b32(rvx, off, 0, 0));
        vy[u] = __uint_as_float(__builtin_amdgcn_raw_buffer_load_b32(rvy, off, 0, 0));
      }
    }
#pragma unroll
    for (int u = 0; u < 4; ++u) {
      const int n = n0 + lane + 64 * u;
      float x = gx[u], y = gy[u];
      if constexpr (VEL) {
        x = __fadd_rn(x, __fmul_rn(tdt, __fmul_rn(vx[u], P.dt32)));
        y = __fadd_rn(y, __fmul_rn(tdt, __fmul_rn(vy[u], P.dt32)));
      }
      const float dx = x - F.tx, dy = y - F.ty;
      const float p0x = fmaf(F.c, dx, F.s * dy), p0y = fmaf(F.c, dy, -(F.s * dx));
      unsigned k = __float_as_uint(geo_key_t<E, RECT>(P, p0x, p0y));
      k = n < n_use ? k : 0xFFFFFFFFu;
      dkey[n] = k;
      lmin = min(lmin, k);
    }
  }
  return lmin;
}

#define SEL2_TRIP 256
#ifdef NPA_SEL_PROF
#define SELP_WAVES 4096
__device__ unsigned long long npa_sel_prof[SELP_WAVES][16];
extern "C" int npa_dbg_sel_prof(unsigned long long* out16, int reset) {
  static unsigned long long host[SELP_WAVES][16];
  if (out16) {
    if (hipMemcpyFromSymbol(host, HIP_SYMBOL(npa_sel_prof), sizeof(host)) != hipSuccess) return -1;
    for (int i = 0; i < 16; ++i) { out16[i] = 0; for (int w = 0; w < SELP_WAVES; ++w) out16[i] += host[w][i]; }
  }
  if (reset) {
    memset(host, 0, sizeof(host));
    if (hipMemcpyToSymbol(HIP_SYMBOL(npa_sel_prof), host, sizeof(host)) != hipSuccess) return -1;
  }
  return 0;
}
#define SELP_DECL unsigned long long spt_ = __builtin_amdgcn_s_memtime(), sacc_[11] = {0, 0, 0, 0, 0, 0, 0, 0, 0, 0, 0}; const unsigned long long sp0_ = spt_
#define SELP(i) do { const unsigned long long n_ = __builtin_amdgcn_s_memtime(); sacc_[i] += n_ - spt_; spt_ = n_; } while (0)
#else
#define SELP_DECL
#define SELP(i)
#endif
template <int E, bool BF16 = false, bool KEYS16 = false>
__global__ __attribute__((amdgpu_flat_work_group_size(64, 64), amdgpu_waves_per_eu(E <= 6 ? 4 : 3, E <= 6 ? 4 : 3))) void select_geo_kernel(
    DevParams P, const float* __restrict__ wpack, int n_stride, const float* __restrict__ cur_s,
    const float* __restrict__ points, const float* __restrict__ vel, const int* __restrict__ n_points,
    const int* __restrict__ flags, float* __restrict__ mu_sorted, float* __restrict__ lam_sorted,
    float* __restrict__ pts_sorted, float* __restrict__ dist_sorted, int* __restrict__ count, int scene0, int t0, int nsl,
    int nscene, int debug, unsigned* __restrict__ stats, const float* __restrict__ trig, unsigned* __restrict__ audit,
    unsigned audit_thresh, unsigned audit_seed, float margin_scale) {
#include "select_geo_carve.inc"
  const int lane = threadIdx.x, j = lane & 31, hf = lane >> 5;
  SELP_DECL;
  const int w = blockIdx.x, xcd = w & 7, r_ = w >> 3;
  const int bl = (r_ / nsl) * 8 + xcd;
  if (bl >= nscene) return;
  const int t = r_ % nsl + t0, b = bl + scene0;
#include "select_geo_body.inc"
}

template <int E, bool BF16 = false, bool KEYS16 = false>
__global__ __attribute__((amdgpu_flat_work_group_size(64, 64), amdgpu_waves_per_eu(E <= 6 ? 4 : 3, E <= 6 ? 4 : 3))) void select_geo_group_kernel(
    DevParams P, SelGeoGroup G, int t0, int nsl, int nscene, int debug, unsigned audit_thresh, float margin_scale) {
  const SelGeoCall& q = G.c[blockIdx.y];
  const float* __restrict__ wpack = q.wpack; const float* __restrict__ cur_s = q.cur_s; const float* __restrict__ points = q.points;
  const float* __restrict__ vel = q.vel; const int* __restrict__ n_points = q.n_points; const int* __restrict__ flags = q.flags;
  float* __restrict__ mu_sorted = q.mu_sorted; float* __restrict__ lam_sorted = q.lam_sorted; float* __restrict__ pts_sorted = q.pts_sorted;
  float* __restrict__ dist_sorted = q.dist_sorted; int* __restrict__ count = q.count; unsigned* __restrict__ stats = q.stats;
  const float* __restrict__ trig = q.trig; unsigned* __restrict__ audit = q.audit;
  const int n_stride = q.n_stride;
  unsigned audit_seed = q.audit_seed;
#include "select_geo_carve.inc"
  const int lane = threadIdx.x, j = lane & 31, hf = lane >> 5;
  SELP_DECL;
  const int w = blockIdx.x, xcd = w & 7, r_ = w >> 3;
  const int bl = (r_ / nsl) * 8 + xcd;
  if (bl >= nscene) return;
  const int t = r_ % nsl + t0, b = bl;
#include "select_geo_body.inc"
}
```

neupan_amd/csrc/select_geo_body.inc:

```
  const int T = P.T, M = P.M;
  constexpr bool TILE16 = !BF16 && !KEYS16;
  if (flags && flags[b * 4 + 0]) return;
  int n_raw = n_points ? n_points[b] : n_stride;
  n_raw = n_raw < 0 ? 0 : (n_raw > n_stride ? n_stride : n_raw);
  const int n_use = n_raw < P.dune_max_num ? n_raw : P.dune_max_num;
  const size_t orow = (size_t)b * (T + 1) + t;
  if (n_use <= 0) {
    if (lane == 0) count[orow] = 0;
    return;
  }
  constexpr int NVEC = 11 * 32 + 8 * 32 + 8, NVT = (NVEC + 63) / 64, NGT = (NPA_GEO_BANDS + 63) / 64;
  float pre_v[NVT], pre_g[NGT];
#pragma unroll
  for (int i = 0; i < NVT; ++i) { const int k = lane + 64 * i; pre_v[i] = wpack[(TILE16 ? WP_VEC16 : WP_VEC) + (k < NVEC ? k : NVEC - 1)]; }
#pragma unroll
  for (int i = 0; i < NGT; ++i) { const int k = lane + 64 * i; pre_g[i] = wpack[WP_GEO + (k < NPA_GEO_BANDS ? k : NPA_GEO_BANDS - 1)]; }
  unsigned aud_viol = 0, aud_launches = 0;
  if (audit) {
    aud_viol = __hip_atomic_load(audit + 2, __ATOMIC_RELAXED, __HIP_MEMORY_SCOPE_AGENT);
    aud_launches = __hip_atomic_load(audit + 4, __ATOMIC_RELAXED, __HIP_MEMORY_SCOPE_AGENT);
  }
  const float w1 = wpack[WP_W1 + lane];
  const float w1a = TILE16 ? wpack[WP_W116 + lane] : 0.f, w1b = TILE16 ? wpack[WP_W116 + 64 + lane] : 0.f;
  SliceFrame F;
  load_frame<E>(P, cur_s, trig, b, t, F);
  const float* px_row = points + (size_t)b * 2 * n_stride;
  const float* py_row = px_row + n_stride;
  const float* vx_row = vel ? vel + (size_t)b * 2 * n_stride : nullptr;
  const float* vy_row = vel ? vx_row + n_stride : nullptr;
  const bool has_vel = vel != nullptr, decim = n_use < n_raw;
  const bool distrust = audit && __builtin_amdgcn_readfirstlane((int)aud_viol) != 0;
  const float boxS = (P.geo_rect && E == 4) ? 0.f : __uint_as_float(__builtin_amdgcn_readfirstlane(__float_as_uint(wpack[WP_TABH + 4])));
  const unsigned far_thr = __float_as_uint(fmaxf(P.geo_far - boxS, 0.f));
  SELP(0);

  const int n_pad = (n_use + SEL2_TRIP - 1) & ~(SEL2_TRIP - 1);
  unsigned lmin;
#define KP(R_, V_, D_) lmin = key_pass<E, R_, V_, D_>(P, F, px_row, py_row, vx_row, vy_row, dkey, n_raw, n_use, n_pad, lane)
  if (has_vel) { if (decim) KP(true, true, true); else KP(true, true, false); }
  else { if (decim) KP(true, false, true); else KP(true, false, false); }
#undef KP
#pragma unroll
  for (int i = 0; i < NVT; ++i) { const int k = lane + 64 * i; if (k < NVEC) smem[k] = pre_v[i]; }
#pragma unroll
  for (int i = 0; i < NGT; ++i) { const int k = lane + 64 * i; if (k < NPA_GEO_BANDS) etab[k] = pre_g[i] * margin_scale; }
  const float* wls = wpack + (BF16 ? WP_WB16 : WP_WLS);
  const float* wls16 = wpack + WP_WL16;
  WSYNC();
  SELP(1);

  const int msel = n_use < M ? n_use : M;
  unsigned bound = 0;
  for (int bit = 31; bit >= 12; --bit) {
    const unsigned trial = bound | ((1u << bit) - 1u);
    if (__popcll(__ballot(lmin <= trial)) < msel) bound |= 1u << bit;
  }
  bound |= 0xFFFu;
  float hi = 0.f;
  if (lmin <= bound) {
    const float g = __uint_as_float(lmin);
    if (lmin >= far_thr) hi = __builtin_inff();
    else {
      float mm = 0.f;
      for (int bb = npa_geo_band(g), be = npa_geo_band(g + boxS); bb <= be; ++bb) mm = fmaxf(mm, etab[bb]);
      hi = g + boxS + mm;
    }
  }
  const float U = wave_max_f32(hi);
  unsigned thr = 0xFFFFFFFEu;
  if (!distrust && U < 3.0e38f) {
    float gs = 0.f;
#pragma unroll
    for (int rep = 0; rep < 2; ++rep) {
      const int bnd = lane + 64 * rep;
      if (bnd < NPA_GEO_BANDS) {
        const float lo_b = __uint_as_float((unsigned)(bnd + (0x3E800000u >> 20)) << 20) - 0.25f;
        const float hi_b = bnd == NPA_GEO_BANDS - 1 ? P.geo_far : __uint_as_float((unsigned)(bnd + 1 + (0x3E800000u >> 20)) << 20) - 0.25f;
        const float reach = U + etab[bnd];
        if (lo_b < P.geo_far && lo_b <= reach) gs = fmaxf(gs, fminf(hi_b, reach));
      }
    }
    gs = wave_max_f32(gs);
    thr = gs < 3.0e38f ? __float_as_uint(gs) : 0xFFFFFFFEu;
  }
  SELP(2);
  int ntot = 0;
  for (int n0 = 0; n0 < n_pad; n0 += SEL2_TRIP) {
    const uint4 k4 = *reinterpret_cast<const uint4*>(dkey + n0 + 4 * lane);
    const unsigned kk[4] = {k4.x, k4.y, k4.z, k4.w};
    bool hit[4];
#pragma unroll
    for (int u = 0; u < 4; ++u) hit[u] = kk[u] <= thr || (kk[u] - far_thr) < (0xFFFFFFFFu - far_thr);
#pragma unroll
    for (int u = 0; u < 4; ++u) {
      const unsigned long long bal = __ballot(hit[u]);
      const int pos = ntot + __builtin_amdgcn_mbcnt_hi((unsigned)(bal >> 32), __builtin_amdgcn_mbcnt_lo((unsigned)bal, 0));
      if (hit[u]) dkey[pos] = (unsigned)(n0 + 4 * lane + u);
      ntot += __popcll(bal);
    }
  }
  WSYNC();
  SELP(3);
  int ncand = ntot, fellback = 0;
  bool overflow = false, all = false;
  int total = 0;
  if (ntot <= SEL_CAP && ntot >= msel) {
    if (lane < ntot) sel[lane] = (int)dkey[lane];
    WSYNC();
  } else if (ntot < msel) {
    overflow = true; fellback = 1; all = true; total = n_use;
  } else {
    overflow = true;
    fellback = 1;
    all = 2 * ntot > n_use;
    total = all ? n_use : ntot;
  }
  unsigned* ckey = dkey + ntot;
  auto cand_index = [&](int q) { return all ? q : (int)dkey[q]; };
  auto extract = [&]() {
    for (int m = 0; m < msel; ++m) {
      unsigned long long best = ~0ull;
      for (int n = lane; n < n_use; n += 64) best = umin64(best, ((unsigned long long)dkey[n] << 32) | (unsigned)n);
      best = wave_min_u64(best);
      const int idx = (int)(best & 0xFFFFFFFFu);
      if (lane == 0) { sel[m] = idx; skey[m] = (unsigned)(best >> 32); dkey[idx] = 0xFFFFFFFFu; }
      WSYNC();
    }
  };
  bool audit_wave = false;
  if (audit && audit_thresh) {
    audit_seed += (unsigned)__builtin_amdgcn_readfirstlane((int)aud_launches);
    if (blockIdx.x == 0 && lane == 0) atomicAdd(audit + 4, 1u);
    unsigned hsh = (audit_seed * 0x9E3779B1u) ^ ((unsigned)b * 0x85EBCA77u) ^ ((unsigned)t * 0xC2B2AE3Du);
    hsh ^= hsh >> 15; hsh *= 0x2C1B3C6Du; hsh ^= hsh >> 12; hsh *= 0x297A2D39u; hsh ^= hsh >> 15;
    audit_wave = hsh < audit_thresh || audit_thresh == 0xFFFFFFFFu;
  }
  int viol = 0;
  float worst = 0.f;
  bool use16 = KEYS16 && overflow && !all && !distrust && total > 128;
  constexpr bool TABF = !BF16 && !KEYS16 && (E == 4 || E == 8);
  bool useT = TABF && P.geo_tab != 0 && !distrust && ntot >= msel && (overflow || ntot > 32);
  if (useT && !overflow) total = ntot;
  bool aud16 = false;
  float m16 = 0.f;
  SELP(4);
#pragma unroll 1
  for (int stage = (overflow || useT) ? 0 : 1;;) {
    const int cnt = stage == 0 ? total : (stage == 1 ? ncand : (n_use < 32 ? n_use : 32));
    if (TABF && stage == 0 && useT) {
      unsigned* fk = all ? dkey : ckey;
#pragma unroll 1
      for (int q0 = 0; q0 < cnt; q0 += 64) {
        const int q = q0 + lane, qc = q < cnt ? q : cnt - 1;
        const int src = src_index(cand_index(qc), n_raw, n_use);
        float gx = px_row[src], gy = py_row[src];
        if (vx_row) {
          gx = __fadd_rn(gx, __fmul_rn(F.tstep, __fmul_rn(vx_row[src], P.dt32)));
          gy = __fadd_rn(gy, __fmul_rn(F.tstep, __fmul_rn(vy_row[src], P.dt32)));
        }
        const float dx = __fsub_rn(gx, F.tx), dy = __fsub_rn(gy, F.ty);
        const float p0x = fmaf(F.c, dx, __fmul_rn(F.s, dy)), p0y = fmaf(F.c, dy, -__fmul_rn(F.s, dx));
        const float gk = geo_key<E>(P, p0x, p0y);
        const unsigned kc = gk < P.geo_far ? ordered_key(gk + geo_tab_corr(wpack, p0x, p0y)) : NPA_TAB_KEY_FAR;
        if (q < cnt) fk[q] = kc;
      }
    } else
#pragma unroll 1
    for (int q0 = 0, tw = 32; q0 < cnt; q0 += tw) {
      const bool narrow = TILE16 && cnt - q0 <= 16;
      tw = narrow ? 16 : 32;
      const bool own = lane < tw;
      const int q = q0 + (lane & (tw - 1)), qc = q < cnt ? q : cnt - 1;
      int idx;
      if (stage == 0) idx = cand_index(qc);
      else if (stage == 1) idx = sel[qc];
      else {
        const int step = n_use >> 5;
        idx = step > 0 ? qc * step + (int)((audit_seed + (unsigned)t) % (unsigned)step) : qc;
      }
      float mu[E], gx, gy, lx, ly, dist, p0x, p0y;
      if constexpr (KEYS16) {
        if (stage == 0 && use16)
          point_features_stream<E, true>(P, F, w1, wpack + WP_WB16, vec, w6, b6, px_row, py_row, vx_row, vy_row,
                                         src_index(idx, n_raw, n_use), lane, mu, gx, gy, lx, ly, dist, p0x, p0y);
        else
          point_features_stream<E, false>(P, F, w1, wls, vec, w6, b6, px_row, py_row, vx_row, vy_row,
                                          src_index(idx, n_raw, n_use), lane, mu, gx, gy, lx, ly, dist, p0x, p0y);
      } else if constexpr (TILE16) {
        if (narrow)
          point_features_stream16<E>(P, F, w1a, w1b, wls16, vec, w6, b6, px_row, py_row, vx_row, vy_row,
                                     src_index(idx, n_raw, n_use), lane, mu, gx, gy, lx, ly, dist, p0x, p0y);
        else
          point_features_stream<E, false, true>(P, F, w1, wls, vec, w6, b6, px_row, py_row, vx_row, vy_row,
                                                src_index(idx, n_raw, n_use), lane, mu, gx, gy, lx, ly, dist, p0x, p0y);
      } else
      point_features_stream<E, BF16>(P, F, w1, wls, vec, w6, b6, px_row, py_row, vx_row, vy_row,
                               src_index(idx, n_raw, n_use), lane, mu, gx, gy, lx, ly, dist, p0x, p0y);
      if constexpr (KEYS16 || TABF) {
        if (stage == 1 && aud16) {
          const unsigned k16 = s16[qc];
          const float d16 = __uint_as_float((k16 & 0x80000000u) ? (k16 & 0x7FFFFFFFu) : ~k16);
          const float ex = fabsf(dist - d16) - (TABF ? wpack[WP_KTAB + npa_geo_band(d16)] * margin_scale : m16);
          const bool bad = own && q < cnt && ex > 0.f;
          viol += bad ? 1 : 0;
          worst = bad ? fmaxf(worst, ex) : worst;
        }
      }
      if (stage != 0 && audit) {
        const float g = geo_key<E>(P, p0x, p0y);
        const float ex = fabsf(dist - g) - etab[npa_geo_band(g)];
        const bool bad = own && q < cnt && g < P.geo_far && ex > 0.f;
        viol += bad ? 1 : 0;
        worst = bad ? fmaxf(worst, ex) : worst;
        if constexpr (TABF) {
          if (audit_wave && P.geo_tab != 0) {
            const float tk = g + geo_tab_corr(wpack, p0x, p0y);
            const float mt = wpack[WP_KTAB + npa_geo_band(tk)] * margin_scale;
            const float ext = fabsf(dist - tk) - mt;
            const bool badt = own && q < cnt && g < P.geo_far && mt < 3.0e38f && ext > 0.f;
            viol += badt ? 1 : 0;
            worst = badt ? fmaxf(worst, ext) : worst;
          }
        }
      }
      if (own && q < cnt) {
        const unsigned k = ordered_key(dist);
        if (stage == 0) {
          if (all) dkey[idx] = k;
          else ckey[q] = k;
        } else if (stage == 1) {
          float* r = rows + q * ROW_W;
#pragma unroll
          for (int e = 0; e < E; ++e) r[e] = mu[e];
          r[E] = lx; r[E + 1] = ly; r[E + 2] = gx; r[E + 3] = gy; r[E + 4] = dist;
          rkey[2 * q] = (unsigned)idx; rkey[2 * q + 1] = k;
        }
      }
    }
    WSYNC();
    if (stage == 0) SELP(5); else if (stage == 1) SELP(6); else SELP(7);
    if (stage == 2) break;
    if (stage == 1) {
      const bool mine = lane < ncand;
      const unsigned long long kx = mine ? (((unsigned long long)rkey[2 * lane + 1] << 32) | rkey[2 * lane]) : ~0ull;
      int rank = 0;
      for (int i = 0; i < ncand; i += 4) {
        const unsigned long long k0 = readlane_u64(kx, i), k1 = readlane_u64(kx, (i + 1) & 63), k2 = readlane_u64(kx, (i + 2) & 63),
                                 k3 = readlane_u64(kx, (i + 3) & 63);
        rank += (k0 < kx ? 1 : 0) + (k1 < kx ? 1 : 0) + (k2 < kx ? 1 : 0) + (k3 < kx ? 1 : 0);
      }
      if (mine && rank < msel) {
        const float* r = rows + lane * ROW_W;
        auto put = [&](int q) {
          const size_t o = orow * M + q;
#pragma unroll
          for (int e = 0; e < E; ++e) mu_sorted[o * E + e] = r[e];
          lam_sorted[o * 2 + 0] = r[E]; lam_sorted[o * 2 + 1] = r[E + 1];
          pts_sorted[o * 2 + 0] = r[E + 2]; pts_sorted[o * 2 + 1] = r[E + 3];
          dist_sorted[o] = r[E + 4];
        };
        put(rank);
        if (rank == 0)
          for (int q = msel; q < M; ++q) put(q);
      }
      if (lane == 0) count[orow] = debug ? (msel | ((ntot < 255 ? ntot : 255) << 8) | (fellback << 16)) : msel;
      SELP(8);
      if (!audit_wave) break;
      stage = 2;
      continue;
    }
    const bool filt = (KEYS16 && use16) || (TABF && useT);
    if (stats && lane == 0 && !(TABF && useT)) atomicAdd(stats, (unsigned)((total + 31) / 32));
    if (all && !filt) {
      extract();
    } else if (filt) {
      const unsigned* fk = all ? dkey : ckey;
      auto key_float = [](unsigned k) { return __uint_as_float((k & 0x80000000u) ? (k & 0x7FFFFFFFu) : ~k); };
      float kt0 = 0.f, kt1 = 0.f, Ub = -3.0e38f;
      if constexpr (TABF) {
        kt0 = wpack[WP_KTAB + lane] * margin_scale;
        kt1 = wpack[WP_KTAB + 64 + (lane < NPA_GEO_BANDS - 64 ? lane : NPA_GEO_BANDS - 65)] * margin_scale;
      }
      unsigned long long prev = 0ull;
      for (int m2 = 0; m2 < msel; ++m2) {
        unsigned long long best = ~0ull;
        for (int q = lane; q < total; q += 64) {
          const unsigned long long v = ((unsigned long long)fk[q] << 32) | (unsigned)cand_index(q);
          if (v < best && (m2 == 0 || v > prev)) best = v;
        }
        prev = wave_min_u64(best);
        if constexpr (TABF) {
          const float km = key_float((unsigned)(prev >> 32));
          const int bm = __builtin_amdgcn_readfirstlane(npa_geo_band(km));
          const float mb = __uint_as_float(bm < 64 ? __builtin_amdgcn_readlane(__float_as_uint(kt0), bm & 63)
                                                   : __builtin_amdgcn_readlane(__float_as_uint(kt1), bm & 63));
          Ub = fmaxf(Ub, km + mb);
          if (!(km == km)) Ub = __builtin_inff();
        }
      }
      const unsigned kth = (unsigned)(prev >> 32);
      const float dk = key_float(kth);
      bool bound_ok;
      unsigned thr16, thr_hi = NPA_TAB_KEY_FAR;
      if constexpr (TABF) {
        float gs = -3.0e38f;
        unsigned long long noinf[2];
#pragma unroll
        for (int rep = 0; rep < 2; ++rep) {
          const int bnd = lane + 64 * rep;
          const float mb = rep == 0 ? kt0 : kt1;
          const bool have = bnd < NPA_GEO_BANDS && mb < 3.0e38f;
          noinf[rep] = __ballot(bnd < NPA_GEO_BANDS && !have);
          if (have) {
            const float lo_b = bnd == 0 ? -3.0e38f : __uint_as_float((unsigned)(bnd + (0x3E800000u >> 20)) << 20) - 0.25f;
            const float hi_b = bnd == NPA_GEO_BANDS - 1 ? 3.0e38f : __uint_as_float((unsigned)(bnd + 1 + (0x3E800000u >> 20)) << 20) - 0.25f;
            const float reach = Ub + mb;
            if (lo_b <= reach) gs = fmaxf(gs, fminf(hi_b, reach));
          }
        }
        gs = wave_max_f32(gs);
        const int binf = noinf[0] ? __builtin_ctzll(noinf[0]) : (noinf[1] ? 64 + __builtin_ctzll(noinf[1]) : NPA_GEO_BANDS);
        const float lo_inf = binf >= NPA_GEO_BANDS ? 3.0e38f
                                                   : (binf == 0 ? -3.0e38f : __uint_as_float((unsigned)(binf + (0x3E800000u >> 20)) << 20) - 0.25f);
        bound_ok = Ub == Ub && Ub < 3.0e38f && gs < lo_inf && gs >= dk;
        thr16 = ordered_key(gs);
        thr_hi = binf >= NPA_GEO_BANDS ? NPA_TAB_KEY_FAR : ordered_key(lo_inf);
        m16 = 0.f;
      } else {
        float mm = 0.f;
        const int b0 = npa_geo_band(dk);
#pragma unroll
        for (int o = -1; o <= 3; ++o) {
          const int bb = b0 + o < 0 ? 0 : (b0 + o >= NPA_GEO_BANDS ? NPA_GEO_BANDS - 1 : b0 + o);
          mm = fmaxf(mm, wpack[WP_K16 + bb]);
        }
        m16 = mm * margin_scale;
        bound_ok = dk == dk && fabsf(dk) < 3.0e38f && m16 < 0.25f;
        thr16 = ordered_key(dk + 2.0f * m16);
      }
      use16 = false; useT = false;
      bool decided = false;
      if (bound_ok) {
        int nsurv = 0;
        for (int q0 = 0; q0 < total; q0 += 64) {
          const int q = q0 + lane;
          const unsigned kq = q < total ? fk[q] : 0xFFFFFFFFu;
          const int iq = q < total ? cand_index(q) : 0;
          const bool hit = q < total && (kq <= thr16 || (TABF && kq >= thr_hi));
          const unsigned long long bal = __ballot(hit);
          const int pos = nsurv + __builtin_amdgcn_mbcnt_hi((unsigned)(bal >> 32), __builtin_amdgcn_mbcnt_lo((unsigned)bal, 0));
          if (hit) {
            dkey[pos] = (unsigned)iq;
            if (pos < SEL_CAP) { sel[pos] = iq; s16[pos] = kq; }
          }
          nsurv += __popcll(bal);
        }
        WSYNC();
        decided = true;
        if (nsurv <= SEL_CAP && nsurv >= msel) {
          fellback = 3;
          aud16 = true;
          all = false;
          ncand = nsurv;
          stage = 1;
          SELP(9);
          continue;
        }
        if (nsurv >= msel) {
          fellback = 2;
          if (!all) total = nsurv;
          else if (2 * nsurv <= n_use) { all = false; total = nsurv; ckey = dkey + nsurv; }
          else total = n_use;
        } else if (all) total = n_use;
      }
      if (!decided && !overflow) {
        if (lane < ntot) sel[lane] = (int)dkey[lane];
        WSYNC();
        ncand = ntot;
        stage = 1;
        continue;
      }
      continue;
    } else {
      int mywin = 0;
      for (int m2 = 0; m2 < msel; ++m2) {
        unsigned long long best = ~0ull;
        int bq = -1;
        for (int q = lane; q < total; q += 64) {
          const unsigned long long v = ((unsigned long long)ckey[q] << 32) | (unsigned)cand_index(q);
          if (v < best) { best = v; bq = q; }
        }
        const unsigned long long win = wave_min_u64(best);
        if (best == win && bq >= 0) ckey[bq] = 0xFFFFFFFFu;
        if (lane == m2) mywin = (int)(win & 0xFFFFFFFFu);
        WSYNC();
      }
      if (lane < msel) sel[lane] = mywin;
      WSYNC();
    }
    ncand = msel;
    stage = 1;
    SELP(9);
  }
  if (audit) {
    const unsigned long long vb = __ballot(viol > 0);
    if (vb != 0ull) {
      int v = viol;
      float wv = worst;
      for (int o = 32; o > 0; o >>= 1) { v += __shfl_xor(v, o, 64); wv = fmaxf(wv, __shfl_xor(wv, o, 64)); }
      if (lane == 0) {
        atomicAdd(audit + 2, (unsigned)v); atomicMax(audit + 3, __float_as_uint(wv));
        unsigned* hp = *reinterpret_cast<unsigned* const*>(audit + 6);
        if (hp) __hip_atomic_fetch_add(hp, (unsigned)v, __ATOMIC_RELAXED, __HIP_MEMORY_SCOPE_SYSTEM);
      }
    }
    if (audit_wave && lane == 0) { atomicAdd(audit + 0, 1u); atomicAdd(audit + 1, (unsigned)(n_use < 32 ? n_use : 32)); }
  }
  SELP(10);
#ifdef NPA_SEL_PROF
  if (lane == 0 && blockIdx.x < SELP_WAVES) {
    unsigned long long* row = npa_sel_prof[blockIdx.x];
    row[15] += 1ull;
    row[14] += (unsigned long long)__builtin_amdgcn_s_memtime() - sp0_;
#pragma unroll
    for (int i = 0; i < 11; ++i) row[i] += sacc_[i];
  }
#endif
```

neupan_amd/csrc/select_geo_carve.inc:

```
  extern __shared__ __attribute__((aligned(16))) float smem[];
  float* vec = smem;
  float* w6 = vec + 11 * 32;
  float* b6 = w6 + 8 * 32;
  float* etab = b6 + 8;
  int* sel = reinterpret_cast<int*>(etab + NPA_GEO_BANDS);
  unsigned* skey = reinterpret_cast<unsigned*>(sel + SEL_CAP);
  constexpr int ROW_W = E + 5;
  unsigned* s16 = skey + NPA_MAX_M;
  unsigned* dkey = s16 + SEL_CAP;
  float* rows = reinterpret_cast<float*>(dkey);
  unsigned* rkey = reinterpret_cast<unsigned*>(rows + SEL_CAP * (NPA_MAX_E + 5));
```

Before: 830,800 plans/s.

## Cut SGPR/VGPR pressure in select_geo by spilling frame to LDS and lazy kernarg loads

The per-slice frame (rotated G rows, G, h, pose) is kept in LDS instead of uniform registers. Kernel arguments such as output pointers, stats, audit and debug are re-read from the kernarg segment when needed rather than held live across the kernel. Boolean state is packed into one bitfield, and fmaxf/ReLU are replaced by fmed3-based max without NaN canonicalisation. The aim is lower register pressure in the selection kernel, at the cost of extra LDS/scalar loads, fragile offsetof-mirrored kernarg layouts, and changed NaN semantics in max.

```diff
diff --git a/neupan_amd/csrc/dune.hip b/neupan_amd/csrc/dune.hip
--- a/neupan_amd/csrc/dune.hip
+++ b/neupan_amd/csrc/dune.hip
@@ -130,7 +130,7 @@
   if (n_use_max < 1) n_use_max = 1;
   const size_t n_pad = ((size_t)n_use_max + SEL2_TRIP - 1) / SEL2_TRIP * SEL2_TRIP;
   const size_t key_area = std::max<size_t>(n_pad * sizeof(unsigned), SEL_CAP * (NPA_MAX_E + 5 + 2) * sizeof(float));
-  const size_t shmem = (11 * 32 + 8 * 32 + 8 + NPA_GEO_BANDS) * sizeof(float) + (2 * SEL_CAP + NPA_MAX_M) * sizeof(int) +
+  const size_t shmem = (11 * 32 + 8 * 32 + 8 + NPA_GEO_BANDS + SEL_LDS_FRAME) * sizeof(float) + (2 * SEL_CAP + NPA_MAX_M) * sizeof(int) +
                        (key_area + 15) / 16 * 16;
   const int blocks = (batch + 7) / 8 * 8 * nsl;
 #define LAUNCHG(EE, BB, KK)                                                                                         \
@@ -182,7 +182,7 @@
   if (n_use_max < 1) n_use_max = 1;
   const size_t n_pad = ((size_t)n_use_max + SEL2_TRIP - 1) / SEL2_TRIP * SEL2_TRIP;
   const size_t key_area = std::max<size_t>(n_pad * sizeof(unsigned), SEL_CAP * (NPA_MAX_E + 5 + 2) * sizeof(float));
-  const size_t shmem = (11 * 32 + 8 * 32 + 8 + NPA_GEO_BANDS) * sizeof(float) + (2 * SEL_CAP + NPA_MAX_M) * sizeof(int) +
+  const size_t shmem = (11 * 32 + 8 * 32 + 8 + NPA_GEO_BANDS + SEL_LDS_FRAME) * sizeof(float) + (2 * SEL_CAP + NPA_MAX_M) * sizeof(int) +
                        (key_area + 15) / 16 * 16;
   const int blocks = (batch + 7) / 8 * 8 * nsl;
 #define LAUNCHG(EE, BB, KK)                                                                                         \
diff --git a/neupan_amd/csrc/dune_device.h b/neupan_amd/csrc/dune_device.h
--- a/neupan_amd/csrc/dune_device.h
+++ b/neupan_amd/csrc/dune_device.h
@@ -101,6 +101,11 @@
   }
 }
 
+__device__ __forceinline__ float inf_reg() { float v = __builtin_inff(); asm("" : "+v"(v)); return v; }
+__device__ __forceinline__ float max_nc(float a, float b) { return __builtin_amdgcn_fmed3f(a, b, inf_reg()); }
+__device__ __forceinline__ float min_nc(float a, float b) { return -__builtin_amdgcn_fmed3f(-a, -b, inf_reg()); }
+__device__ __forceinline__ float relu_acc(float x) { return max_nc(x, 0.f); }
+
 __device__ __forceinline__ f32x16 layer32(const float (&w)[16], const float (&a)[16], f32x16 acc) {
 #pragma unroll
   for (int r = 0; r < 16; ++r) acc = __builtin_amdgcn_mfma_f32_32x32x2f32(w[r], a[r], acc, 0, 0, 0);
@@ -306,7 +311,7 @@
   {
     f32x16 acc = layer32(wa, a, bias_init<PERM>(vec + V_B2 * 32, hf));
 #pragma unroll
-    for (int r = 0; r < 16; ++r) a[r] = fmaxf(acc[r], 0.f);
+    for (int r = 0; r < 16; ++r) a[r] = relu_acc(acc[r]);
   }
   __builtin_amdgcn_sched_barrier(0);
   load_layer(wls, 2, lane, wa);
@@ -321,7 +326,7 @@
   {
     f32x16 acc = layer32(wa, a, bias_init<PERM>(vec + V_B4 * 32, hf));
 #pragma unroll
-    for (int r = 0; r < 16; ++r) a[r] = fmaxf(acc[r], 0.f);
+    for (int r = 0; r < 16; ++r) a[r] = relu_acc(acc[r]);
   }
   __builtin_amdgcn_sched_barrier(0);
   {
@@ -397,7 +402,7 @@
     f32x4 c0 = ld4(vq + V_B2 * 32), c1 = ld4(vq + V_B2 * 32 + 4);
     layer16(wa, a, c0, c1);
 #pragma unroll
-    for (int r = 0; r < 4; ++r) { a[r] = fmaxf(c0[r], 0.f); a[4 + r] = fmaxf(c1[r], 0.f); }
+    for (int r = 0; r < 4; ++r) { a[r] = relu_acc(c0[r]); a[4 + r] = relu_acc(c1[r]); }
   }
   __builtin_amdgcn_sched_barrier(0);
   load_layer(wls16, 2, lane, wa);
@@ -414,7 +419,7 @@
     f32x4 c0 = ld4(vq + V_B4 * 32), c1 = ld4(vq + V_B4 * 32 + 4);
     layer16(wa, a, c0, c1);
 #pragma unroll
-    for (int r = 0; r < 4; ++r) { a[r] = fmaxf(c0[r], 0.f); a[4 + r] = fmaxf(c1[r], 0.f); }
+    for (int r = 0; r < 4; ++r) { a[r] = relu_acc(c0[r]); a[4 + r] = relu_acc(c1[r]); }
   }
   __builtin_amdgcn_sched_barrier(0);
   {
@@ -463,7 +468,7 @@
   {
     f32x16 acc = layer32_bf16(wb, 0, lane, a, bias_init(vec + V_B2 * 32, hf));
 #pragma unroll
-    for (int r = 0; r < 16; ++r) a[r] = fmaxf(acc[r], 0.f);
+    for (int r = 0; r < 16; ++r) a[r] = relu_acc(acc[r]);
   }
   {
     f32x16 acc = layer32_bf16(wb, 1, lane, a, bias_init(vec + V_B3 * 32, hf));
@@ -472,7 +477,7 @@
   {
     f32x16 acc = layer32_bf16(wb, 2, lane, a, bias_init(vec + V_B4 * 32, hf));
 #pragma unroll
-    for (int r = 0; r < 16; ++r) a[r] = fmaxf(acc[r], 0.f);
+    for (int r = 0; r < 16; ++r) a[r] = relu_acc(acc[r]);
   }
   {
     f32x16 acc = layer32_bf16(wb, 3, lane, a, bias_init(vec + V_B5 * 32, hf));
@@ -527,9 +532,9 @@
   return (int)((double)n * step);
 }
 
-template <int E>
+template <int E, bool RG_LDS = false>
 __device__ __forceinline__ void load_frame(const DevParams& P, const float* __restrict__ cur_s,
-                                           const float* __restrict__ trig, int b, int t, SliceFrame& F) {
+                                           const float* __restrict__ trig, int b, int t, SliceFrame& F, float* frg = nullptr) {
   const int T = P.T;
   const float* s = cur_s + (size_t)b * 3 * (T + 1);
   F.tx = s[t];
@@ -543,9 +548,22 @@
     F.rg[1][e] = fmaf(-F.s, P.G[e][0], -__fmul_rn(F.c, P.G[e][1]));
   }
   auto uni = [](float v) { return __uint_as_float(__builtin_amdgcn_readfirstlane(__float_as_uint(v))); };
+  if constexpr (RG_LDS) {
+    if (threadIdx.x == 0) {
+#pragma unroll
+      for (int e = 0; e < E; ++e) {
+        frg[e] = F.rg[0][e]; frg[NPA_MAX_E + e] = F.rg[1][e];
+        frg[2 * NPA_MAX_E + e] = P.G[e][0]; frg[3 * NPA_MAX_E + e] = P.G[e][1]; frg[4 * NPA_MAX_E + e] = P.h[e];
+      }
+      frg[5 * NPA_MAX_E + 0] = F.c; frg[5 * NPA_MAX_E + 1] = F.s; frg[5 * NPA_MAX_E + 2] = F.tx; frg[5 * NPA_MAX_E + 3] = F.ty;
+      frg[5 * NPA_MAX_E + 4] = F.tstep;
+    }
+  }
   F.c = uni(F.c); F.s = uni(F.s); F.tx = uni(F.tx); F.ty = uni(F.ty); F.tstep = uni(F.tstep);
-#pragma unroll
-  for (int e = 0; e < E; ++e) { F.rg[0][e] = uni(F.rg[0][e]); F.rg[1][e] = uni(F.rg[1][e]); }
+  if constexpr (!RG_LDS) {
+#pragma unroll
+    for (int e = 0; e < E; ++e) { F.rg[0][e] = uni(F.rg[0][e]); F.rg[1][e] = uni(F.rg[1][e]); }
+  }
 }
 
 template <int E, int SPLIT>
@@ -575,31 +593,21 @@
   }
 }
 
-template <int E, bool BF16 = false, bool PERM = false>
-__device__ __forceinline__ void point_features_stream(const DevParams& P, const SliceFrame& F, float w1, const float* __restrict__ wls,
-                                                      const float* vec, const float* w6, const float* b6, const float* px_row,
-                                                      const float* py_row, const float* vx_row, const float* vy_row, int src,
-                                                      int lane, float mu[E], float& gx, float& gy, float& lx, float& ly,
-                                                      float& dist, float& p0x, float& p0y) {
-  gx = px_row[src];
-  gy = py_row[src];
-  if (vx_row) {
-    gx = __fadd_rn(gx, __fmul_rn(F.tstep, __fmul_rn(vx_row[src], P.dt32)));
-    gy = __fadd_rn(gy, __fmul_rn(F.tstep, __fmul_rn(vy_row[src], P.dt32)));
-  }
-  float dx = __fsub_rn(gx, F.tx), dy = __fsub_rn(gy, F.ty);
+__device__ __forceinline__ float wpack_at(const float* __restrict__ wpack, int i) { asm("" : "+v"(i)); return wpack[i]; }
+__device__ __forceinline__ void slice_point(const DevParams& P, const SliceFrame& F, const float* __restrict__ pts,
+                                            const float* __restrict__ vel, int n_stride, int src, float& gx, float& gy,
+                                            float& p0x, float& p0y) {
+  int sy = src + n_stride;
+  asm("" : "+v"(sy));
+  gx = pts[src];
+  gy = pts[sy];
+  if (vel) {
+    gx = __fadd_rn(gx, __fmul_rn(F.tstep, __fmul_rn(vel[src], P.dt32)));
+    gy = __fadd_rn(gy, __fmul_rn(F.tstep, __fmul_rn(vel[sy], P.dt32)));
+  }
+  const float dx = __fsub_rn(gx, F.tx), dy = __fsub_rn(gy, F.ty);
   p0x = fmaf(F.c, dx, __fmul_rn(F.s, dy));
   p0y = fmaf(F.c, dy, -__fmul_rn(F.s, dx));
-  if constexpr (BF16) encode_tile_bf16<E>(w1, wls, vec, w6, b6, p0x, p0y, lane, mu);
-  else encode_tile_stream<E, PERM>(w1, wls, vec, w6, b6, p0x, p0y, lane, mu);
-  lx = 0.f; ly = 0.f; dist = 0.f;
-#pragma unroll
-  for (int e = 0; e < E; ++e) {
-    lx = fmaf(F.rg[0][e], mu[e], lx);
-    ly = fmaf(F.rg[1][e], mu[e], ly);
-    float tmp = __fsub_rn(fmaf(P.G[e][0], p0x, __fmul_rn(P.G[e][1], p0y)), P.h[e]);
-    dist = fmaf(mu[e], tmp, dist);
-  }
 }
 
 template <int E>
@@ -988,15 +996,15 @@
 
 __device__ __forceinline__ float dpp_f32_b1(float v) { return __int_as_float(__builtin_amdgcn_update_dpp(0, __float_as_int(v), 0xB1, 0xF, 0xF, false)); }
 __device__ __forceinline__ float wave_max_f32(float v) {
-  v = fmaxf(v, dpp_f32_b1(v));
-  v = fmaxf(v, __int_as_float(__builtin_amdgcn_update_dpp(0, __float_as_int(v), 0x4E, 0xF, 0xF, false)));
-  v = fmaxf(v, __int_as_float(__builtin_amdgcn_update_dpp(0, __float_as_int(v), 0x141, 0xF, 0xF, false)));
-  v = fmaxf(v, __int_as_float(__builtin_amdgcn_update_dpp(0, __float_as_int(v), 0x140, 0xF, 0xF, false)));
+  v = max_nc(v, dpp_f32_b1(v));
+  v = max_nc(v, __int_as_float(__builtin_amdgcn_update_dpp(0, __float_as_int(v), 0x4E, 0xF, 0xF, false)));
+  v = max_nc(v, __int_as_float(__builtin_amdgcn_update_dpp(0, __float_as_int(v), 0x141, 0xF, 0xF, false)));
+  v = max_nc(v, __int_as_float(__builtin_amdgcn_update_dpp(0, __float_as_int(v), 0x140, 0xF, 0xF, false)));
   auto rl = [&](int l) { return __uint_as_float(__builtin_amdgcn_readlane(__float_as_uint(v), l)); };
-  return fmaxf(fmaxf(rl(0), rl(16)), fmaxf(rl(32), rl(48)));
-}
-template <int E, bool RECT>
-__device__ __forceinline__ float geo_key_t(const DevParams& P, float x, float y) {
+  return max_nc(max_nc(rl(0), rl(16)), max_nc(rl(32), rl(48)));
+}
+template <int E, bool RECT, class PP>
+__device__ __forceinline__ float geo_key_t(const PP& P, float x, float y) {
   if constexpr (RECT) {
     const float dx = fmaxf(fabsf(x - P.rcx) - P.rhx, 0.f), dy = fmaxf(fabsf(y - P.rcy) - P.rhy, 0.f);
     return __builtin_amdgcn_sqrtf(fmaf(dx, dx, dy * dy));
@@ -1015,8 +1023,8 @@
     return inside ? 0.f : __builtin_amdgcn_sqrtf(best);
   }
 }
-template <int E>
-__device__ __forceinline__ float geo_key(const DevParams& P, float x, float y) {
+template <int E, class PP>
+__device__ __forceinline__ float geo_key(const PP& P, float x, float y) {
   return P.geo_rect ? geo_key_t<E, true>(P, x, y) : geo_key_t<E, false>(P, x, y);
 }
 
@@ -1084,6 +1092,12 @@
   return lmin;
 }
 
+#define SEL_OPAQUE_V(x) asm volatile("" : "+v"(x))
+#define SEL_OPAQUE_S(x) do { (x) = __builtin_amdgcn_readfirstlane(x); asm volatile("" : "+s"(x)); } while (0)
+#define SEL_LDS_FRAME (6 * NPA_MAX_E)
+enum { ST_OVERFLOW = 1, ST_ALL = 2, ST_USE16 = 4, ST_USET = 8, ST_AUD16 = 16, ST_AUDIT_WAVE = 32, ST_HAS_AUDIT = 64, ST_DISTRUST = 128 };
+#define ST_IS(f) ((st & (unsigned)(f)) != 0u)
+#define ST_PUT(f, v) (st = (v) ? (st | (unsigned)(f)) : (st & ~(unsigned)(f)))
 #define SEL2_TRIP 256
 #ifdef NPA_SEL_PROF
 #define SELP_WAVES 4096
@@ -1106,41 +1120,95 @@
 #define SELP_DECL
 #define SELP(i)
 #endif
+#define NPA_KARG __attribute__((address_space(4)))
+#define NPA_GLOBAL __attribute__((address_space(1)))
+typedef const char NPA_KARG* karg_ptr;
+struct SelGeoArgs {
+  DevParams P; const float* wpack; int n_stride; const float* cur_s; const float* points; const float* vel; const int* n_points;
+  const int* flags; float* mu_sorted; float* lam_sorted; float* pts_sorted; float* dist_sorted; int* count; int scene0, t0, nsl,
+  nscene, debug; unsigned* stats; const float* trig; unsigned* audit; unsigned audit_thresh, audit_seed; float margin_scale;
+};
+struct SelGeoGroupArgs { DevParams P; SelGeoGroup G; int t0, nsl, nscene, debug; unsigned audit_thresh; float margin_scale; };
+struct SelOutPtrs { float* mu; float* lam; float* pts; float* dist; int* count; };
+static_assert(offsetof(SelGeoArgs, count) - offsetof(SelGeoArgs, mu_sorted) == 32 && offsetof(SelGeoCall, count) - offsetof(SelGeoCall, mu_sorted) == 32,
+              "SelOutPtrs is read as one block");
+static_assert(sizeof(DevParams) == 0x1a8 && offsetof(SelGeoArgs, wpack) == sizeof(DevParams) && offsetof(SelGeoGroupArgs, G) == sizeof(DevParams),
+              "DevParams is the first argument of both kernels");
+static_assert(sizeof(SelGeoCall) == 0x78 && sizeof(SelGeoGroupArgs) == 0x1a8 + 8 * 0x78 + 24 && offsetof(SelGeoGroupArgs, debug) == 0x1a8 + 8 * 0x78 + 12,
+              "SelGeoGroupArgs mirrors select_geo_group_kernel(P, G, t0, nsl, nscene, debug, audit_thresh, margin_scale)");
+static_assert(offsetof(SelGeoArgs, mu_sorted) == 0x1a8 + 0x38 && offsetof(SelGeoArgs, debug) == 0x1a8 + 0x70 && offsetof(SelGeoArgs, stats) == 0x1a8 + 0x78 &&
+              offsetof(SelGeoArgs, audit) == 0x1a8 + 0x88 && sizeof(SelGeoArgs) == 0x1a8 + 0xa0,
+              "SelGeoArgs mirrors the parameter list of select_geo_kernel");
+__device__ __forceinline__ karg_ptr karg_fence(karg_ptr p) { asm volatile("" : "+s"(p)); return p; }
+template <class T>
+__device__ __forceinline__ T karg_load(karg_ptr p, size_t off) { return *reinterpret_cast<const T NPA_KARG*>(p + off); }
+#define SEL_KARG(T_, member) karg_load<T_>(SEL_KARGS_LATE(), SEL_KARG_OFF(member))
+template <int E>
+__device__ __forceinline__ float geo_key_karg(karg_ptr kbase, float x, float y) {
+  return geo_key<E>(*reinterpret_cast<const DevParams NPA_KARG*>(karg_fence(kbase)), x, y);
+}
+
 template <int E, bool BF16 = false, bool KEYS16 = false>
 __global__ __attribute__((amdgpu_flat_work_group_size(64, 64), amdgpu_waves_per_eu(E <= 6 ? 4 : 3, E <= 6 ? 4 : 3))) void select_geo_kernel(
     DevParams P, const float* __restrict__ wpack, int n_stride, const float* __restrict__ cur_s,
     const float* __restrict__ points, const float* __restrict__ vel, const int* __restrict__ n_points,
-    const int* __restrict__ flags, float* __restrict__ mu_sorted, float* __restrict__ lam_sorted,
-    float* __restrict__ pts_sorted, float* __restrict__ dist_sorted, int* __restrict__ count, int scene0, int t0, int nsl,
-    int nscene, int debug, unsigned* __restrict__ stats, const float* __restrict__ trig, unsigned* __restrict__ audit,
+    const int* __restrict__ flags, float* __restrict__ mu_sorted_, float* __restrict__ lam_sorted_,
+    float* __restrict__ pts_sorted_, float* __restrict__ dist_sorted_, int* __restrict__ count_, int scene0, int t0, int nsl,
+    int nscene, int debug, unsigned* __restrict__ stats_, const float* __restrict__ trig, unsigned* __restrict__ audit,
     unsigned audit_thresh, unsigned audit_seed, float margin_scale) {
+#define SEL_KARG_OFF(member) offsetof(SelGeoArgs, member)
+#define SEL_KBASE_OFF(member) offsetof(SelGeoArgs, member)
+  const karg_ptr sel_kbase = (karg_ptr)__builtin_amdgcn_kernarg_segment_ptr();
+#define SEL_KARGS_LATE() karg_fence(sel_kbase)
+#define SEL_KOFF_STORE()
+#define SEL_KOFF() 0
 #include "select_geo_carve.inc"
-  const int lane = threadIdx.x, j = lane & 31, hf = lane >> 5;
+  int lane = threadIdx.x;
   SELP_DECL;
   const int w = blockIdx.x, xcd = w & 7, r_ = w >> 3;
   const int bl = (r_ / nsl) * 8 + xcd;
   if (bl >= nscene) return;
   const int t = r_ % nsl + t0, b = bl + scene0;
 #include "select_geo_body.inc"
+#undef SEL_KARG_OFF
+#undef SEL_KBASE_OFF
+#undef SEL_KARGS_LATE
+#undef SEL_KOFF_STORE
+#undef SEL_KOFF
 }
 
 template <int E, bool BF16 = false, bool KEYS16 = false>
 __global__ __attribute__((amdgpu_flat_work_group_size(64, 64), amdgpu_waves_per_eu(E <= 6 ? 4 : 3, E <= 6 ? 4 : 3))) void select_geo_group_kernel(
     DevParams P, SelGeoGroup G, int t0, int nsl, int nscene, int debug, unsigned audit_thresh, float margin_scale) {
-  const SelGeoCall& q = G.c[blockIdx.y];
-  const float* __restrict__ wpack = q.wpack; const float* __restrict__ cur_s = q.cur_s; const float* __restrict__ points = q.points;
-  const float* __restrict__ vel = q.vel; const int* __restrict__ n_points = q.n_points; const int* __restrict__ flags = q.flags;
-  float* __restrict__ mu_sorted = q.mu_sorted; float* __restrict__ lam_sorted = q.lam_sorted; float* __restrict__ pts_sorted = q.pts_sorted;
-  float* __restrict__ dist_sorted = q.dist_sorted; int* __restrict__ count = q.count; unsigned* __restrict__ stats = q.stats;
-  const float* __restrict__ trig = q.trig; unsigned* __restrict__ audit = q.audit;
-  const int n_stride = q.n_stride;
-  unsigned audit_seed = q.audit_seed;
+#define SEL_KARG_OFF(member) offsetof(SelGeoCall, member)
+#define SEL_KBASE_OFF(member) offsetof(SelGeoGroupArgs, member)
+  const karg_ptr sel_kbase = (karg_ptr)__builtin_amdgcn_kernarg_segment_ptr();
+  const int sel_koff = (int)offsetof(SelGeoGroupArgs, G) + (int)blockIdx.y * (int)sizeof(SelGeoCall);
+  const karg_ptr sel_kargs = sel_kbase + sel_koff;
+#define SEL_KARGS_LATE() (karg_fence(sel_kbase) + __builtin_amdgcn_readfirstlane(__float_as_int(frg[5 * NPA_MAX_E + 7])))
+#define SEL_KOFF_STORE() do { if (threadIdx.x == 0) frg[5 * NPA_MAX_E + 7] = __int_as_float(sel_koff); } while (0)
+#define SEL_KOFF() sel_koff
+  const float* __restrict__ wpack = karg_load<const float*>(sel_kargs, SEL_KARG_OFF(wpack));
+  const float* __restrict__ cur_s = karg_load<const float*>(sel_kargs, SEL_KARG_OFF(cur_s));
+  const float* __restrict__ points = karg_load<const float*>(sel_kargs, SEL_KARG_OFF(points));
+  const float* __restrict__ vel = karg_load<const float*>(sel_kargs, SEL_KARG_OFF(vel));
+  const int* __restrict__ n_points = karg_load<const int*>(sel_kargs, SEL_KARG_OFF(n_points));
+  const int* __restrict__ flags = karg_load<const int*>(sel_kargs, SEL_KARG_OFF(flags));
+  const float* __restrict__ trig = karg_load<const float*>(sel_kargs, SEL_KARG_OFF(trig));
+  unsigned* __restrict__ audit = karg_load<unsigned*>(sel_kargs, SEL_KARG_OFF(audit));
+  const int n_stride = karg_load<int>(sel_kargs, SEL_KARG_OFF(n_stride));
+  unsigned audit_seed = karg_load<unsigned>(sel_kargs, SEL_KARG_OFF(audit_seed));
 #include "select_geo_carve.inc"
-  const int lane = threadIdx.x, j = lane & 31, hf = lane >> 5;
+  int lane = threadIdx.x;
   SELP_DECL;
   const int w = blockIdx.x, xcd = w & 7, r_ = w >> 3;
   const int bl = (r_ / nsl) * 8 + xcd;
   if (bl >= nscene) return;
   const int t = r_ % nsl + t0, b = bl;
 #include "select_geo_body.inc"
-}
+#undef SEL_KARG_OFF
+#undef SEL_KBASE_OFF
+#undef SEL_KARGS_LATE
+#undef SEL_KOFF_STORE
+#undef SEL_KOFF
+}
diff --git a/neupan_amd/csrc/select_geo_body.inc b/neupan_amd/csrc/select_geo_body.inc
--- a/neupan_amd/csrc/select_geo_body.inc
+++ b/neupan_amd/csrc/select_geo_body.inc
@@ -3,10 +3,14 @@
   if (flags && flags[b * 4 + 0]) return;
   int n_raw = n_points ? n_points[b] : n_stride;
   n_raw = n_raw < 0 ? 0 : (n_raw > n_stride ? n_stride : n_raw);
-  const int n_use = n_raw < P.dune_max_num ? n_raw : P.dune_max_num;
-  const size_t orow = (size_t)b * (T + 1) + t;
+  int n_use = n_raw < P.dune_max_num ? n_raw : P.dune_max_num;
+  int orow_v = b;
+  asm volatile("" : "+v"(orow_v));
+  orow_v = orow_v * (T + 1) + t;
+  int koff_v = SEL_KOFF();
+  asm volatile("" : "+v"(koff_v));
   if (n_use <= 0) {
-    if (lane == 0) count[orow] = 0;
+    if (lane == 0) ((int NPA_GLOBAL*)karg_load<int*>(karg_fence(sel_kbase) + __builtin_amdgcn_readfirstlane(koff_v), SEL_KARG_OFF(count)))[orow_v] = 0;
     return;
   }
   constexpr int NVEC = 11 * 32 + 8 * 32 + 8, NVT = (NVEC + 63) / 64, NGT = (NPA_GEO_BANDS + 63) / 64;
@@ -23,20 +27,22 @@
   const float w1 = wpack[WP_W1 + lane];
   const float w1a = TILE16 ? wpack[WP_W116 + lane] : 0.f, w1b = TILE16 ? wpack[WP_W116 + 64 + lane] : 0.f;
   SliceFrame F;
-  load_frame<E>(P, cur_s, trig, b, t, F);
+  load_frame<E, true>(P, cur_s, trig, b, t, F, frg);
+  if (lane == 0) frg[5 * NPA_MAX_E + 5] = __int_as_float(orow_v);
+  SEL_KOFF_STORE();
   const float* px_row = points + (size_t)b * 2 * n_stride;
-  const float* py_row = px_row + n_stride;
   const float* vx_row = vel ? vel + (size_t)b * 2 * n_stride : nullptr;
-  const float* vy_row = vel ? vx_row + n_stride : nullptr;
   const bool has_vel = vel != nullptr, decim = n_use < n_raw;
-  const bool distrust = audit && __builtin_amdgcn_readfirstlane((int)aud_viol) != 0;
+  const bool has_audit = audit != nullptr;
+  const bool distrust = has_audit && __builtin_amdgcn_readfirstlane((int)aud_viol) != 0;
   const float boxS = (P.geo_rect && E == 4) ? 0.f : __uint_as_float(__builtin_amdgcn_readfirstlane(__float_as_uint(wpack[WP_TABH + 4])));
   const unsigned far_thr = __float_as_uint(fmaxf(P.geo_far - boxS, 0.f));
   SELP(0);
 
   const int n_pad = (n_use + SEL2_TRIP - 1) & ~(SEL2_TRIP - 1);
   unsigned lmin;
-#define KP(R_, V_, D_) lmin = key_pass<E, R_, V_, D_>(P, F, px_row, py_row, vx_row, vy_row, dkey, n_raw, n_use, n_pad, lane)
+#define KP(R_, V_, D_) \
+  lmin = key_pass<E, R_, V_, D_>(P, F, px_row, px_row + n_stride, vx_row, vx_row ? vx_row + n_stride : nullptr, dkey, n_raw, n_use, n_pad, lane)
   if (has_vel) { if (decim) KP(true, true, true); else KP(true, true, false); }
   else { if (decim) KP(true, false, true); else KP(true, false, false); }
 #undef KP
@@ -49,7 +55,7 @@
   WSYNC();
   SELP(1);
 
-  const int msel = n_use < M ? n_use : M;
+  int msel = n_use < M ? n_use : M;
   unsigned bound = 0;
   for (int bit = 31; bit >= 12; --bit) {
     const unsigned trial = bound | ((1u << bit) - 1u);
@@ -62,7 +68,7 @@
     if (lmin >= far_thr) hi = __builtin_inff();
     else {
       float mm = 0.f;
-      for (int bb = npa_geo_band(g), be = npa_geo_band(g + boxS); bb <= be; ++bb) mm = fmaxf(mm, etab[bb]);
+      for (int bb = npa_geo_band(g), be = npa_geo_band(g + boxS); bb <= be; ++bb) mm = max_nc(mm, etab[bb]);
       hi = g + boxS + mm;
     }
   }
@@ -77,7 +83,7 @@
         const float lo_b = __uint_as_float((unsigned)(bnd + (0x3E800000u >> 20)) << 20) - 0.25f;
         const float hi_b = bnd == NPA_GEO_BANDS - 1 ? P.geo_far : __uint_as_float((unsigned)(bnd + 1 + (0x3E800000u >> 20)) << 20) - 0.25f;
         const float reach = U + etab[bnd];
-        if (lo_b < P.geo_far && lo_b <= reach) gs = fmaxf(gs, fminf(hi_b, reach));
+        if (lo_b < P.geo_far && lo_b <= reach) gs = max_nc(gs, min_nc(hi_b, reach));
       }
     }
     gs = wave_max_f32(gs);
@@ -102,21 +108,21 @@
   WSYNC();
   SELP(3);
   int ncand = ntot, fellback = 0;
-  bool overflow = false, all = false;
+  unsigned st = (has_audit ? (unsigned)ST_HAS_AUDIT : 0u) | (distrust ? (unsigned)ST_DISTRUST : 0u);
   int total = 0;
   if (ntot <= SEL_CAP && ntot >= msel) {
     if (lane < ntot) sel[lane] = (int)dkey[lane];
     WSYNC();
   } else if (ntot < msel) {
-    overflow = true; fellback = 1; all = true; total = n_use;
+    ST_PUT(ST_OVERFLOW, true); fellback = 1; ST_PUT(ST_ALL, true); total = n_use;
   } else {
-    overflow = true;
+    ST_PUT(ST_OVERFLOW, true);
     fellback = 1;
-    all = 2 * ntot > n_use;
-    total = all ? n_use : ntot;
+    ST_PUT(ST_ALL, 2 * ntot > n_use);
+    total = ST_IS(ST_ALL) ? n_use : ntot;
   }
   unsigned* ckey = dkey + ntot;
-  auto cand_index = [&](int q) { return all ? q : (int)dkey[q]; };
+  auto cand_index = [&](int q) { return ST_IS(ST_ALL) ? q : (int)dkey[q]; };
   auto extract = [&]() {
     for (int m = 0; m < msel; ++m) {
       unsigned long long best = ~0ull;
@@ -127,40 +133,39 @@
       WSYNC();
     }
   };
-  bool audit_wave = false;
   if (audit && audit_thresh) {
     audit_seed += (unsigned)__builtin_amdgcn_readfirstlane((int)aud_launches);
     if (blockIdx.x == 0 && lane == 0) atomicAdd(audit + 4, 1u);
     unsigned hsh = (audit_seed * 0x9E3779B1u) ^ ((unsigned)b * 0x85EBCA77u) ^ ((unsigned)t * 0xC2B2AE3Du);
     hsh ^= hsh >> 15; hsh *= 0x2C1B3C6Du; hsh ^= hsh >> 12; hsh *= 0x297A2D39u; hsh ^= hsh >> 15;
-    audit_wave = hsh < audit_thresh || audit_thresh == 0xFFFFFFFFu;
+    ST_PUT(ST_AUDIT_WAVE, hsh < audit_thresh || audit_thresh == 0xFFFFFFFFu);
+    if (lane == 0) frg[5 * NPA_MAX_E + 6] = __uint_as_float(audit_seed + (unsigned)t);
   }
   int viol = 0;
   float worst = 0.f;
-  bool use16 = KEYS16 && overflow && !all && !distrust && total > 128;
+  ST_PUT(ST_USE16, KEYS16 && ST_IS(ST_OVERFLOW) && !ST_IS(ST_ALL) && !ST_IS(ST_DISTRUST) && total > 128);
   constexpr bool TABF = !BF16 && !KEYS16 && (E == 4 || E == 8);
-  bool useT = TABF && P.geo_tab != 0 && !distrust && ntot >= msel && (overflow || ntot > 32);
-  if (useT && !overflow) total = ntot;
-  bool aud16 = false;
+  ST_PUT(ST_USET, TABF && P.geo_tab != 0 && !ST_IS(ST_DISTRUST) && ntot >= msel && (ST_IS(ST_OVERFLOW) || ntot > 32));
+  if (ST_IS(ST_USET) && !ST_IS(ST_OVERFLOW)) total = ntot;
+  ST_PUT(ST_AUD16, false);
   float m16 = 0.f;
   SELP(4);
 #pragma unroll 1
-  for (int stage = (overflow || useT) ? 0 : 1;;) {
+  for (int stage = (ST_IS(ST_OVERFLOW) || ST_IS(ST_USET)) ? 0 : 1;;) {
+    SEL_OPAQUE_V(lane); SEL_OPAQUE_S(n_use); SEL_OPAQUE_S(n_raw); SEL_OPAQUE_S(msel);
     const int cnt = stage == 0 ? total : (stage == 1 ? ncand : (n_use < 32 ? n_use : 32));
-    if (TABF && stage == 0 && useT) {
-      unsigned* fk = all ? dkey : ckey;
+    if (TABF && stage == 0 && ST_IS(ST_USET)) {
+      unsigned* fk = ST_IS(ST_ALL) ? dkey : ckey;
 #pragma unroll 1
       for (int q0 = 0; q0 < cnt; q0 += 64) {
         const int q = q0 + lane, qc = q < cnt ? q : cnt - 1;
         const int src = src_index(cand_index(qc), n_raw, n_use);
-        float gx = px_row[src], gy = py_row[src];
-        if (vx_row) {
-          gx = __fadd_rn(gx, __fmul_rn(F.tstep, __fmul_rn(vx_row[src], P.dt32)));
-          gy = __fadd_rn(gy, __fmul_rn(F.tstep, __fmul_rn(vy_row[src], P.dt32)));
-        }
-        const float dx = __fsub_rn(gx, F.tx), dy = __fsub_rn(gy, F.ty);
-        const float p0x = fmaf(F.c, dx, __fmul_rn(F.s, dy)), p0y = fmaf(F.c, dy, -__fmul_rn(F.s, dx));
-        const float gk = geo_key<E>(P, p0x, p0y);
+        SliceFrame Fl;
+        Fl.c = frg[5 * NPA_MAX_E + 0]; Fl.s = frg[5 * NPA_MAX_E + 1];
+        Fl.tx = frg[5 * NPA_MAX_E + 2]; Fl.ty = frg[5 * NPA_MAX_E + 3]; Fl.tstep = frg[5 * NPA_MAX_E + 4];
+        float gx, gy, p0x, p0y;
+        slice_point(P, Fl, px_row, vx_row, n_stride, src, gx, gy, p0x, p0y);
+        const float gk = geo_key_karg<E>(sel_kbase, p0x, p0y);
         const unsigned kc = gk < P.geo_far ? ordered_key(gk + geo_tab_corr(wpack, p0x, p0y)) : NPA_TAB_KEY_FAR;
         if (q < cnt) fk[q] = kc;
       }
@@ -176,57 +181,59 @@
       else if (stage == 1) idx = sel[qc];
       else {
         const int step = n_use >> 5;
-        idx = step > 0 ? qc * step + (int)((audit_seed + (unsigned)t) % (unsigned)step) : qc;
-      }
-      float mu[E], gx, gy, lx, ly, dist, p0x, p0y;
+        idx = step > 0 ? qc * step + (int)(__float_as_uint(frg[5 * NPA_MAX_E + 6]) % (unsigned)step) : qc;
+      }
+      float mu[E], gx, gy, lx = 0.f, ly = 0.f, dist = 0.f, p0x, p0y;
+      SliceFrame Fl;
+      Fl.c = frg[5 * NPA_MAX_E + 0]; Fl.s = frg[5 * NPA_MAX_E + 1];
+      Fl.tx = frg[5 * NPA_MAX_E + 2]; Fl.ty = frg[5 * NPA_MAX_E + 3]; Fl.tstep = frg[5 * NPA_MAX_E + 4];
+      slice_point(P, Fl, px_row, vx_row, n_stride, src_index(idx, n_raw, n_use), gx, gy, p0x, p0y);
       if constexpr (KEYS16) {
-        if (stage == 0 && use16)
-          point_features_stream<E, true>(P, F, w1, wpack + WP_WB16, vec, w6, b6, px_row, py_row, vx_row, vy_row,
-                                         src_index(idx, n_raw, n_use), lane, mu, gx, gy, lx, ly, dist, p0x, p0y);
-        else
-          point_features_stream<E, false>(P, F, w1, wls, vec, w6, b6, px_row, py_row, vx_row, vy_row,
-                                          src_index(idx, n_raw, n_use), lane, mu, gx, gy, lx, ly, dist, p0x, p0y);
+        if (stage == 0 && ST_IS(ST_USE16)) encode_tile_bf16<E>(w1, wpack + WP_WB16, vec, w6, b6, p0x, p0y, lane, mu);
+        else encode_tile_stream<E, false>(w1, wls, vec, w6, b6, p0x, p0y, lane, mu);
       } else if constexpr (TILE16) {
-        if (narrow)
-          point_features_stream16<E>(P, F, w1a, w1b, wls16, vec, w6, b6, px_row, py_row, vx_row, vy_row,
-                                     src_index(idx, n_raw, n_use), lane, mu, gx, gy, lx, ly, dist, p0x, p0y);
-        else
-          point_features_stream<E, false, true>(P, F, w1, wls, vec, w6, b6, px_row, py_row, vx_row, vy_row,
-                                                src_index(idx, n_raw, n_use), lane, mu, gx, gy, lx, ly, dist, p0x, p0y);
-      } else
-      point_features_stream<E, BF16>(P, F, w1, wls, vec, w6, b6, px_row, py_row, vx_row, vy_row,
-                               src_index(idx, n_raw, n_use), lane, mu, gx, gy, lx, ly, dist, p0x, p0y);
+        if (narrow) encode_tile16_stream<E>(w1a, w1b, wls16, vec, w6, b6, p0x, p0y, lane, mu);
+        else encode_tile_stream<E, true>(w1, wls, vec, w6, b6, p0x, p0y, lane, mu);
+      } else if constexpr (BF16) encode_tile_bf16<E>(w1, wls, vec, w6, b6, p0x, p0y, lane, mu);
+      else encode_tile_stream<E, false>(w1, wls, vec, w6, b6, p0x, p0y, lane, mu);
+#pragma unroll
+      for (int e = 0; e < E; ++e) {
+        lx = fmaf(frg[e], mu[e], lx);
+        ly = fmaf(frg[NPA_MAX_E + e], mu[e], ly);
+        const float tmp = __fsub_rn(fmaf(frg[2 * NPA_MAX_E + e], p0x, __fmul_rn(frg[3 * NPA_MAX_E + e], p0y)), frg[4 * NPA_MAX_E + e]);
+        dist = fmaf(mu[e], tmp, dist);
+      }
       if constexpr (KEYS16 || TABF) {
-        if (stage == 1 && aud16) {
+        if (stage == 1 && ST_IS(ST_AUD16)) {
           const unsigned k16 = s16[qc];
           const float d16 = __uint_as_float((k16 & 0x80000000u) ? (k16 & 0x7FFFFFFFu) : ~k16);
-          const float ex = fabsf(dist - d16) - (TABF ? wpack[WP_KTAB + npa_geo_band(d16)] * margin_scale : m16);
+          const float ex = fabsf(dist - d16) - (TABF ? wpack_at(wpack, WP_KTAB + npa_geo_band(d16)) * margin_scale : m16);
           const bool bad = own && q < cnt && ex > 0.f;
           viol += bad ? 1 : 0;
-          worst = bad ? fmaxf(worst, ex) : worst;
-        }
-      }
-      if (stage != 0 && audit) {
-        const float g = geo_key<E>(P, p0x, p0y);
+          worst = bad ? max_nc(worst, ex) : worst;
+        }
+      }
+      if (stage != 0 && ST_IS(ST_HAS_AUDIT)) {
+        const float g = geo_key_karg<E>(sel_kbase, p0x, p0y);
         const float ex = fabsf(dist - g) - etab[npa_geo_band(g)];
         const bool bad = own && q < cnt && g < P.geo_far && ex > 0.f;
         viol += bad ? 1 : 0;
-        worst = bad ? fmaxf(worst, ex) : worst;
+        worst = bad ? max_nc(worst, ex) : worst;
         if constexpr (TABF) {
-          if (audit_wave && P.geo_tab != 0) {
+          if (ST_IS(ST_AUDIT_WAVE) && karg_load<int>(karg_fence(sel_kbase), offsetof(DevParams, geo_tab)) != 0) {
             const float tk = g + geo_tab_corr(wpack, p0x, p0y);
-            const float mt = wpack[WP_KTAB + npa_geo_band(tk)] * margin_scale;
+            const float mt = wpack_at(wpack, WP_KTAB + npa_geo_band(tk)) * margin_scale;
             const float ext = fabsf(dist - tk) - mt;
             const bool badt = own && q < cnt && g < P.geo_far && mt < 3.0e38f && ext > 0.f;
             viol += badt ? 1 : 0;
-            worst = badt ? fmaxf(worst, ext) : worst;
+            worst = badt ? max_nc(worst, ext) : worst;
           }
         }
       }
       if (own && q < cnt) {
         const unsigned k = ordered_key(dist);
         if (stage == 0) {
-          if (all) dkey[idx] = k;
+          if (ST_IS(ST_ALL)) dkey[idx] = k;
           else ckey[q] = k;
         } else if (stage == 1) {
           float* r = rows + q * ROW_W;
@@ -241,8 +248,13 @@
     if (stage == 0) SELP(5); else if (stage == 1) SELP(6); else SELP(7);
     if (stage == 2) break;
     if (stage == 1) {
+      const size_t orow = (size_t)__float_as_int(frg[5 * NPA_MAX_E + 5]);
+      const int Me = karg_load<int>(karg_fence(sel_kbase), offsetof(DevParams, M));
       const bool mine = lane < ncand;
       const unsigned long long kx = mine ? (((unsigned long long)rkey[2 * lane + 1] << 32) | rkey[2 * lane]) : ~0ull;
+      const karg_ptr ko = SEL_KARGS_LATE() + SEL_KARG_OFF(mu_sorted);
+      const SelOutPtrs O = {karg_load<float*>(ko, 0), karg_load<float*>(ko, 8), karg_load<float*>(ko, 16), karg_load<float*>(ko, 24),
+                            karg_load<int*>(ko, 32)};
       int rank = 0;
       for (int i = 0; i < ncand; i += 4) {
         const unsigned long long k0 = readlane_u64(kx, i), k1 = readlane_u64(kx, (i + 1) & 63), k2 = readlane_u64(kx, (i + 2) & 63),
@@ -251,8 +263,10 @@
       }
       if (mine && rank < msel) {
         const float* r = rows + lane * ROW_W;
+        float NPA_GLOBAL* mu_sorted = (float NPA_GLOBAL*)O.mu; float NPA_GLOBAL* lam_sorted = (float NPA_GLOBAL*)O.lam;
+        float NPA_GLOBAL* pts_sorted = (float NPA_GLOBAL*)O.pts; float NPA_GLOBAL* dist_sorted = (float NPA_GLOBAL*)O.dist;
         auto put = [&](int q) {
-          const size_t o = orow * M + q;
+          const size_t o = orow * Me + q;
 #pragma unroll
           for (int e = 0; e < E; ++e) mu_sorted[o * E + e] = r[e];
           lam_sorted[o * 2 + 0] = r[E]; lam_sorted[o * 2 + 1] = r[E + 1];
@@ -261,25 +275,38 @@
         };
         put(rank);
         if (rank == 0)
-          for (int q = msel; q < M; ++q) put(q);
-      }
-      if (lane == 0) count[orow] = debug ? (msel | ((ntot < 255 ? ntot : 255) << 8) | (fellback << 16)) : msel;
+#pragma unroll 1
+          for (int q = msel; q < Me; ++q) put(q);
+      }
+      if (lane == 0) {
+        int word = msel;
+        if (karg_load<int>(karg_fence(sel_kbase), SEL_KBASE_OFF(debug))) {
+          int nt = ntot;
+          asm volatile("" : "+s"(nt));
+          word |= ((nt < 255 ? nt : 255) << 8) | (fellback << 16);
+        }
+        ((int NPA_GLOBAL*)O.count)[orow] = word;
+      }
       SELP(8);
-      if (!audit_wave) break;
+      if (!ST_IS(ST_AUDIT_WAVE)) break;
       stage = 2;
       continue;
     }
-    const bool filt = (KEYS16 && use16) || (TABF && useT);
-    if (stats && lane == 0 && !(TABF && useT)) atomicAdd(stats, (unsigned)((total + 31) / 32));
-    if (all && !filt) {
+    SEL_OPAQUE_S(st);
+    const bool filt = (KEYS16 && ST_IS(ST_USE16)) || (TABF && ST_IS(ST_USET));
+    if (lane == 0 && !(TABF && ST_IS(ST_USET))) {
+      unsigned* stats = SEL_KARG(unsigned*, stats);
+      if (stats) atomicAdd(stats, (unsigned)((total + 31) / 32));
+    }
+    if (ST_IS(ST_ALL) && !filt) {
       extract();
     } else if (filt) {
-      const unsigned* fk = all ? dkey : ckey;
+      const unsigned* fk = ST_IS(ST_ALL) ? dkey : ckey;
       auto key_float = [](unsigned k) { return __uint_as_float((k & 0x80000000u) ? (k & 0x7FFFFFFFu) : ~k); };
       float kt0 = 0.f, kt1 = 0.f, Ub = -3.0e38f;
       if constexpr (TABF) {
-        kt0 = wpack[WP_KTAB + lane] * margin_scale;
-        kt1 = wpack[WP_KTAB + 64 + (lane < NPA_GEO_BANDS - 64 ? lane : NPA_GEO_BANDS - 65)] * margin_scale;
+        kt0 = wpack_at(wpack, WP_KTAB + lane) * margin_scale;
+        kt1 = wpack_at(wpack, WP_KTAB + 64 + (lane < NPA_GEO_BANDS - 64 ? lane : NPA_GEO_BANDS - 65)) * margin_scale;
       }
       unsigned long long prev = 0ull;
       for (int m2 = 0; m2 < msel; ++m2) {
@@ -294,7 +321,7 @@
           const int bm = __builtin_amdgcn_readfirstlane(npa_geo_band(km));
           const float mb = __uint_as_float(bm < 64 ? __builtin_amdgcn_readlane(__float_as_uint(kt0), bm & 63)
                                                    : __builtin_amdgcn_readlane(__float_as_uint(kt1), bm & 63));
-          Ub = fmaxf(Ub, km + mb);
+          Ub = max_nc(Ub, km + mb);
           if (!(km == km)) Ub = __builtin_inff();
         }
       }
@@ -315,7 +342,7 @@
             const float lo_b = bnd == 0 ? -3.0e38f : __uint_as_float((unsigned)(bnd + (0x3E800000u >> 20)) << 20) - 0.25f;
             const float hi_b = bnd == NPA_GEO_BANDS - 1 ? 3.0e38f : __uint_as_float((unsigned)(bnd + 1 + (0x3E800000u >> 20)) << 20) - 0.25f;
             const float reach = Ub + mb;
-            if (lo_b <= reach) gs = fmaxf(gs, fminf(hi_b, reach));
+            if (lo_b <= reach) gs = max_nc(gs, min_nc(hi_b, reach));
           }
         }
         gs = wave_max_f32(gs);
@@ -338,7 +365,7 @@
         bound_ok = dk == dk && fabsf(dk) < 3.0e38f && m16 < 0.25f;
         thr16 = ordered_key(dk + 2.0f * m16);
       }
-      use16 = false; useT = false;
+      ST_PUT(ST_USE16, false); ST_PUT(ST_USET, false);
       bool decided = false;
       if (bound_ok) {
         int nsurv = 0;
@@ -359,8 +386,8 @@
         decided = true;
         if (nsurv <= SEL_CAP && nsurv >= msel) {
           fellback = 3;
-          aud16 = true;
-          all = false;
+          ST_PUT(ST_AUD16, true);
+          ST_PUT(ST_ALL, false);
           ncand = nsurv;
           stage = 1;
           SELP(9);
@@ -368,12 +395,12 @@
         }
         if (nsurv >= msel) {
           fellback = 2;
-          if (!all) total = nsurv;
-          else if (2 * nsurv <= n_use) { all = false; total = nsurv; ckey = dkey + nsurv; }
+          if (!ST_IS(ST_ALL)) total = nsurv;
+          else if (2 * nsurv <= n_use) { ST_PUT(ST_ALL, false); total = nsurv; ckey = dkey + nsurv; }
           else total = n_use;
-        } else if (all) total = n_use;
-      }
-      if (!decided && !overflow) {
+        } else if (ST_IS(ST_ALL)) total = n_use;
+      }
+      if (!decided && !ST_IS(ST_OVERFLOW)) {
         if (lane < ntot) sel[lane] = (int)dkey[lane];
         WSYNC();
         ncand = ntot;
@@ -402,19 +429,23 @@
     stage = 1;
     SELP(9);
   }
-  if (audit) {
+  if (ST_IS(ST_HAS_AUDIT)) {
     const unsigned long long vb = __ballot(viol > 0);
     if (vb != 0ull) {
+      unsigned* audit_g = SEL_KARG(unsigned*, audit);
       int v = viol;
       float wv = worst;
-      for (int o = 32; o > 0; o >>= 1) { v += __shfl_xor(v, o, 64); wv = fmaxf(wv, __shfl_xor(wv, o, 64)); }
+      for (int o = 32; o > 0; o >>= 1) { v += __shfl_xor(v, o, 64); wv = max_nc(wv, __shfl_xor(wv, o, 64)); }
       if (lane == 0) {
-        atomicAdd(audit + 2, (unsigned)v); atomicMax(audit + 3, __float_as_uint(wv));
-        unsigned* hp = *reinterpret_cast<unsigned* const*>(audit + 6);
+        atomicAdd(audit_g + 2, (unsigned)v); atomicMax(audit_g + 3, __float_as_uint(wv));
+        unsigned* hp = *reinterpret_cast<unsigned* const*>(audit_g + 6);
         if (hp) __hip_atomic_fetch_add(hp, (unsigned)v, __ATOMIC_RELAXED, __HIP_MEMORY_SCOPE_SYSTEM);
       }
     }
-    if (audit_wave && lane == 0) { atomicAdd(audit + 0, 1u); atomicAdd(audit + 1, (unsigned)(n_use < 32 ? n_use : 32)); }
+    if (ST_IS(ST_AUDIT_WAVE) && lane == 0) {
+      unsigned* audit_g = SEL_KARG(unsigned*, audit);
+      atomicAdd(audit_g + 0, 1u); atomicAdd(audit_g + 1, (unsigned)(n_use < 32 ? n_use : 32));
+    }
   }
   SELP(10);
 #ifdef NPA_SEL_PROF
diff --git a/neupan_amd/csrc/select_geo_carve.inc b/neupan_amd/csrc/select_geo_carve.inc
--- a/neupan_amd/csrc/select_geo_carve.inc
+++ b/neupan_amd/csrc/select_geo_carve.inc
@@ -3,7 +3,8 @@
   float* w6 = vec + 11 * 32;
   float* b6 = w6 + 8 * 32;
   float* etab = b6 + 8;
-  int* sel = reinterpret_cast<int*>(etab + NPA_GEO_BANDS);
+  float* frg = etab + NPA_GEO_BANDS;
+  int* sel = reinterpret_cast<int*>(frg + SEL_LDS_FRAME);
   unsigned* skey = reinterpret_cast<unsigned*>(sel + SEL_CAP);
   constexpr int ROW_W = E + 5;
   unsigned* s16 = skey + NPA_MAX_M;
```

After: 860,100 plans/s (median of 6 runs). 3.5% higher.
